# pwrliang/grpc-rdma

Hardware: NVIDIA B200
Metric: streaming_payload_GBps_256conns_4MiB (higher is better)
Workload: dtype u8

## Files before the change

### grpc-rdma_b200/csrc/b200_dev.cuh

```cuda
#pragma once
#include <stdint.h>

#if defined(__CUDACC__)
#define B200_HD __host__ __device__ __forceinline__
#else
#define B200_HD inline
#endif

namespace b200 {

constexpr uint64_t kAlign = 8;
constexpr uint64_t kReserved = 24;
constexpr uint64_t kFooter = ~0ull;
constexpr int kMaxSgeLimit = 32;

B200_HD uint64_t round_up8(uint64_t v) { return (v + 7) & ~7ull; }
B200_HD uint64_t round_down8(uint64_t v) { return v & ~7ull; }
B200_HD uint64_t encoded_size(uint64_t payload) { return 16 + round_up8(payload); }
B200_HD uint64_t calc_writable(uint64_t space) { return space > kReserved ? round_down8(space - kReserved) : 0; }
B200_HD uint64_t free_size(uint64_t cap, uint64_t head, uint64_t tail) {
  return cap - ((tail + cap - head) & (cap - 1));
}
B200_HD uint64_t writable_size(uint64_t cap, uint64_t head, uint64_t tail) {
  uint64_t f = free_size(cap, head, tail);
  return f > kReserved ? f - kReserved : 0;
}

struct PairMirror {
  uint64_t head, moving_head, remain, acc;
  uint64_t remote_tail, credit_head;
  uint64_t readable;
  uint32_t partial_write;
  uint32_t peer_exit;
  uint32_t has_message;
  uint32_t _reserved;
};

struct __align__(128) PairDev {
  uint8_t* ring;
  uint64_t cap;
  uint8_t* peer_ring;
  uint64_t* peer_credit;
  PairMirror* mirror;
  PairMirror* peer_mirror;
  uint32_t status;
  uint32_t max_sge;
  int32_t peer_slot;
  uint32_t wire;
  uint64_t head;
  uint64_t moving_head;
  uint64_t remain;
  uint64_t acc;
  uint64_t remote_tail;
  uint32_t partial_write;
  uint32_t mlock;
  uint64_t credit_head;
  uint32_t credit_exit;
  uint32_t _pad1;
};
static_assert(sizeof(PairDev) == 128, "PairDev is one 128-byte line");

struct SliceDev {
  const uint8_t* ptr;
  uint64_t len;
};

struct SendOpDev {
  int32_t slot;
  uint32_t flags;
  const SliceDev* slices;
  uint64_t nslices;
  uint64_t byte_idx;
  uint64_t nreal;
};

struct RecvOpDev {
  int32_t slot;
  uint32_t flags;
  uint8_t* dst;
  uint64_t cap;
};

struct OpResult {
  uint64_t bytes;
  uint64_t calls;
};

constexpr uint32_t kFlagUntilBlocked = 0x1;
constexpr uint32_t kFlagConcurrent = 0x8;
constexpr uint32_t kEvReadable = 0x1;
constexpr uint32_t kEvWritable = 0x4;

constexpr uint32_t kStConnected = 2;
constexpr uint32_t kStHalfClosed = 3;
constexpr uint32_t kStError = 5;

constexpr uint32_t kSvcSend = 1, kSvcRecv = 2, kSvcStop = 3, kSvcRetire = 4, kSvcNop = 5;
constexpr uint32_t kSvcInline = 5;
constexpr uint32_t kOwnQ = 16;
constexpr uint32_t kOwnBoxes = 8;
constexpr uint32_t kSmallMax = 8192;
constexpr uint32_t kEagerMax = 2048;
constexpr uint32_t kSvcSliceArea = 1024;
struct __align__(128) SvcCmd {
  uint32_t stamp;
  uint32_t op;
  int32_t slot;
  uint32_t flags;
  uint64_t ptr;
  uint64_t n;
  uint64_t byte_idx;
  SliceDev inl[kSvcInline];
  uint32_t nreal;
  uint32_t stamp2;
};
static_assert(sizeof(SvcCmd) == 128, "one command = one 128-byte line");
struct __align__(16) SvcDone {
  uint64_t bytes;
  uint32_t calls;
  uint32_t seq;
};
static_assert(sizeof(SvcDone) == 16, "one answer = one 16-byte store");
struct PairSvc {
  uint64_t delivered;
  uint64_t pushed_at;
};
struct __align__(32) EagerRec {
  uint64_t at;
  uint64_t csum;
  uint32_t size;
  uint32_t magic;
  uint64_t _pad;
};
constexpr uint32_t kEagerMagic = 0xEA6E7001u;
struct __align__(128) BigBox {
  uint32_t state;
  uint32_t kind;
  int32_t slot;
  uint32_t flags;
  uint64_t ptr, n, byte_idx, nreal;
  SliceDev inl[kSvcInline];
  SvcDone* done;
  uint32_t seq;
  uint32_t _pad;
  OpResult res;
};
B200_HD uint64_t eager_mix(uint64_t x) {
  x ^= x >> 32;
  x *= 0xD6E8FEB86659FD93ull;
  x ^= x >> 32;
  return x;
}
B200_HD uint64_t eager_word(uint64_t w, uint32_t j) { return eager_mix(w + (uint64_t)(j + 1) * 0x9E3779B97F4A7C15ull); }

constexpr uint32_t kReadyRing = 4096;
struct ReadyEntry {
  uint32_t stamp;
  uint16_t slot;
  uint16_t events;
};
struct SvcPollState {
  uint32_t hi_slot;
  uint32_t stop;
  uint32_t ready_next;
  uint32_t scans;
};
struct SvcParams {
  PairDev* pairs;
  PairSvc* psvc;
  SvcCmd* cmds;
  SvcDone* done;
  BigBox* boxes;
  EagerRec* erec;
  uint8_t* eslots;
  SvcPollState* ps;
  uint32_t* last_ev;
  ReadyEntry* ready;
  uint32_t* host_scans;
  int nowners, nbig;
};

void launch_send(PairDev* pairs, const SendOpDev* ops, OpResult* results, int nops, void* stream);
void launch_recv(PairDev* pairs, const RecvOpDev* ops, OpResult* results, int nops, void* stream);
void launch_poll_scan(PairDev* pairs, const int32_t* slots, uint32_t* events, uint32_t* ready_count,
                      int32_t* ready_slots, int n, void* stream);

bool launch_service(const SvcParams& sp, void* s_owner, void* s_big, void* s_poll);
int svc_trace_read(unsigned long long* out16);

void launch_probe_copy(uint8_t* dst, const uint8_t* src, uint64_t bytes_per_cta, uint64_t stride, int nctas,
                       int threads, uint32_t mis, uint32_t item_bytes, uint32_t dynamic, void* stream);

}
```

### grpc-rdma_b200/csrc/b200_kernels.cu

```cuda
#include <cuda_runtime.h>
#include <stdint.h>

#include <mutex>

#include "b200_dev.cuh"

#ifndef B200_RECV_PROXY_FENCE
#define B200_RECV_PROXY_FENCE 1
#endif

namespace b200 {


#define VL(x) (*(volatile decltype(x)*)&(x))

__device__ __forceinline__ uint4 ld_stream16(const void* p) {
  uint4 r;
  asm volatile("ld.global.nc.L1::no_allocate.v4.u32 {%0,%1,%2,%3}, [%4];"
               : "=r"(r.x), "=r"(r.y), "=r"(r.z), "=r"(r.w)
               : "l"(p));
  return r;
}
__device__ __forceinline__ uint4 ld_ring16(const void* p) {
  uint4 r;
  asm volatile("ld.global.L1::no_allocate.v4.u32 {%0,%1,%2,%3}, [%4];"
               : "=r"(r.x), "=r"(r.y), "=r"(r.z), "=r"(r.w)
               : "l"(p));
  return r;
}
__device__ __forceinline__ void st_stream16(void* p, uint4 v) {
  asm volatile("st.global.L1::no_allocate.v4.u32 [%0], {%1,%2,%3,%4};" ::"l"(p), "r"(v.x), "r"(v.y), "r"(v.z),
               "r"(v.w)
               : "memory");
}
__device__ __forceinline__ uint64_t ld_acquire_u64(const void* p) {
  uint64_t v;
  asm volatile("ld.acquire.sys.global.u64 %0, [%1];" : "=l"(v) : "l"(p) : "memory");
  return v;
}
__device__ __forceinline__ uint64_t ld_volatile_u64(const void* p) {
  uint64_t v;
  asm volatile("ld.volatile.global.u64 %0, [%1];" : "=l"(v) : "l"(p) : "memory");
  return v;
}

__device__ __forceinline__ uint32_t ld_acquire_u32(const void* p) {
  uint32_t v;
  asm volatile("ld.acquire.sys.global.u32 %0, [%1];" : "=r"(v) : "l"(p) : "memory");
  return v;
}
__device__ __forceinline__ void st_release_v2u64(void* p, uint64_t a, uint64_t b) {
  __threadfence_system();
  asm volatile("st.global.v2.u64 [%0], {%1,%2};" ::"l"(p), "l"(a), "l"(b) : "memory");
}


__device__ __forceinline__ uint32_t smem_u32(const void* p) { return (uint32_t)__cvta_generic_to_shared(p); }
__device__ __forceinline__ void mbar_init(uint64_t* bar, uint32_t count) {
  asm volatile("mbarrier.init.shared::cta.b64 [%0], %1;" ::"r"(smem_u32(bar)), "r"(count) : "memory");
}
__device__ __forceinline__ void mbar_expect_tx(uint64_t* bar, uint32_t bytes) {
  asm volatile("mbarrier.arrive.expect_tx.shared::cta.b64 _, [%0], %1;" ::"r"(smem_u32(bar)), "r"(bytes) : "memory");
}
__device__ __forceinline__ bool mbar_try_wait(uint64_t* bar, uint32_t parity) {
  uint32_t ok;
  asm volatile(
      "{\n\t.reg .pred p;\n\t"
      "mbarrier.try_wait.parity.shared::cta.b64 p, [%1], %2;\n\t"
      "selp.u32 %0, 1, 0, p;\n\t}"
      : "=r"(ok)
      : "r"(smem_u32(bar)), "r"(parity)
      : "memory");
  return ok != 0;
}
__device__ __forceinline__ void bulk_g2s(void* sdst, const void* gsrc, uint32_t bytes, uint64_t* bar) {
  asm volatile("cp.async.bulk.shared::cluster.global.mbarrier::complete_tx::bytes [%0], [%1], %2, [%3];" ::"r"(
                   smem_u32(sdst)),
               "l"(gsrc), "r"(bytes), "r"(smem_u32(bar))
               : "memory");
}
__device__ __forceinline__ void fence_proxy_async_global() { asm volatile("fence.proxy.async.global;" ::: "memory"); }

template <int K>
__device__ __forceinline__ void s2g_vectors(uint4* __restrict__ dv, const uint4* __restrict__ sv, uint32_t nvec,
                                            uint32_t r, uint32_t lane) {
#pragma unroll 4
  for (uint32_t i = lane; i < nvec; i += 32) {
    const uint4 A = sv[i], B = sv[i + 1];
    uint32_t x0, x1, x2, x3, x4;
    if (K == 0) { x0 = A.x; x1 = A.y; x2 = A.z; x3 = A.w; x4 = B.x; }
    else if (K == 1) { x0 = A.y; x1 = A.z; x2 = A.w; x3 = B.x; x4 = B.y; }
    else if (K == 2) { x0 = A.z; x1 = A.w; x2 = B.x; x3 = B.y; x4 = B.z; }
    else { x0 = A.w; x1 = B.x; x2 = B.y; x3 = B.z; x4 = B.w; }
    uint4 o;
    o.x = __funnelshift_r(x0, x1, r);
    o.y = __funnelshift_r(x1, x2, r);
    o.z = __funnelshift_r(x2, x3, r);
    o.w = __funnelshift_r(x3, x4, r);
    st_stream16(dv + i, o);
  }
}

__device__ __forceinline__ void smem_to_global(uint8_t* dst, const uint8_t* sbase, uint32_t soff, uint32_t n,
                                               uint32_t lane) {
  if (n == 0) return;
  uint32_t head = (16 - (uint32_t)(reinterpret_cast<uintptr_t>(dst) & 15)) & 15;
  if (head > n) head = n;
  const uint32_t nvec = (n - head) >> 4;
  const uint32_t tail = n - head - (nvec << 4);
  if (lane < head) dst[lane] = sbase[soff + lane];
  if (lane < tail) dst[head + (nvec << 4) + lane] = sbase[soff + head + (nvec << 4) + lane];
  const uint32_t vs = soff + head, m = vs & 15;
  const uint4* sv = reinterpret_cast<const uint4*>(sbase + (vs - m));
  uint4* dv = reinterpret_cast<uint4*>(dst + head);
  if (m == 0) {
#pragma unroll 4
    for (uint32_t i = lane; i < nvec; i += 32) st_stream16(dv + i, sv[i]);
    return;
  }
  const uint32_t r = (m & 3) * 8;
  switch (m >> 2) {
    case 0: s2g_vectors<0>(dv, sv, nvec, r, lane); break;
    case 1: s2g_vectors<1>(dv, sv, nvec, r, lane); break;
    case 2: s2g_vectors<2>(dv, sv, nvec, r, lane); break;
    default: s2g_vectors<3>(dv, sv, nvec, r, lane); break;
  }
}

__device__ __forceinline__ void coop_zero(uint8_t* p, uint64_t n, uint32_t lane) {
  if (n == 0) return;
  uint64_t head = (16 - (reinterpret_cast<uintptr_t>(p) & 15)) & 15;
  if (head > n) head = n;
  if (lane < head) p[lane] = 0;
  p += head;
  n -= head;
  const uint64_t nvec = n >> 4;
  uint4* d = reinterpret_cast<uint4*>(p);
  const uint4 z = make_uint4(0, 0, 0, 0);
  for (uint64_t i = lane; i < nvec; i += 32) st_stream16(d + i, z);
  const uint64_t done = nvec << 4;
  if (lane < n - done) p[done + lane] = 0;
}

template <bool kSys = true>
__device__ __forceinline__ void rx_probe(const uint8_t* ring, uint64_t cap, uint64_t head, uint64_t remain,
                                         uint32_t& has_msg, uint64_t& readable) {
  if (remain > 0) {
    has_msg = 1;
    readable = remain;
    return;
  }
  uint64_t hdr = kSys ? ld_acquire_u64(ring + head) : ld_volatile_u64(ring + head);
  has_msg = hdr != 0;
  readable = 0;
  if (hdr != 0 && hdr <= cap - kReserved) {
    const uint8_t* fp = ring + ((head + 8 + round_up8(hdr)) & (cap - 1));
    uint64_t foot = kSys ? ld_acquire_u64(fp) : ld_volatile_u64(fp);
    if (foot == kFooter) readable = hdr;
  }
}

__device__ __forceinline__ void publish_mirror_rx(PairMirror* m, const PairDev* P, uint32_t has_msg,
                                                  uint64_t readable) {
  if (m == nullptr) return;
  volatile PairMirror* vm = m;
  vm->head = P->head;
  vm->moving_head = P->moving_head;
  vm->remain = P->remain;
  vm->acc = P->acc;
  vm->readable = readable;
  vm->has_message = has_msg;
}
__device__ __forceinline__ void publish_mirror_tx(PairMirror* m, const PairDev* P) {
  if (m == nullptr) return;
  volatile PairMirror* vm = m;
  vm->remote_tail = P->remote_tail;
  vm->credit_head = *(volatile const uint64_t*)&P->credit_head;
  vm->partial_write = P->partial_write;
  vm->peer_exit = *(volatile const uint32_t*)&P->credit_exit;
}

__device__ __forceinline__ void mirror_lock(PairDev* P, bool on) {
  if (!on) return;
  while (atomicCAS(&P->mlock, 0u, 1u) != 0u) __nanosleep(64);
  __threadfence();
}
__device__ __forceinline__ void mirror_unlock(PairDev* P, bool on) {
  if (!on) return;
  __threadfence_system();
  atomicExch(&P->mlock, 0u);
}


#ifndef B200_MOVERS
#define B200_MOVERS 8
#endif
#ifndef B200_DEPTH
#define B200_DEPTH 3
#endif
#ifndef B200_CHUNK
#define B200_CHUNK 4096
#endif
constexpr int kMovers = B200_MOVERS;
constexpr int kThreads = 32 * (1 + kMovers);
constexpr int kDepth = B200_DEPTH;
constexpr uint32_t kChunk = B200_CHUNK;
constexpr uint32_t kStageBytes = kChunk + 32;
constexpr uint32_t kStageTotal = kMovers * kDepth * kStageBytes;
constexpr uint32_t kQI = 128;

struct WorkItem {
  uint64_t a;
  uint64_t b;
  uint64_t c;
  uint32_t n;
  uint32_t ready;
};

struct PipeCtl {
  uint32_t next;
  uint32_t total_items;
  uint32_t seg_done;
  uint32_t op_done;
};

__device__ __forceinline__ uint32_t ld_shared_volatile(const uint32_t* p) { return *(const volatile uint32_t*)p; }

__device__ __forceinline__ void publish_item(WorkItem* q, uint32_t id, uint64_t a, uint64_t b, uint64_t c,
                                             uint32_t n) {
  WorkItem* slot = &q[id % kQI];
  while (ld_shared_volatile(&slot->ready) != 0) __nanosleep(20);
  slot->a = a;
  slot->b = b;
  slot->c = c;
  slot->n = n;
  __threadfence_block();
  *(volatile uint32_t*)&slot->ready = id + 1;
}

__device__ __forceinline__ void movers_init(uint64_t* bars, uint32_t tid) {
  if (tid < kMovers * kDepth) mbar_init(&bars[tid], 1);
  asm volatile("fence.mbarrier_init.release.cluster;" ::: "memory");
  asm volatile("fence.proxy.async.shared::cta;" ::: "memory");
}

template <class Move>
__device__ __forceinline__ void mover_run(const Move& mv, WorkItem* q, PipeCtl* ctl, uint8_t* stages, uint64_t* bars,
                                          uint32_t& phase_bits, uint32_t lane) {
  static_assert(kQI <= 256 && kDepth <= 8, "slot_of packs one byte per stage");
  uint32_t head = 0, tail = 0, ticket = 0;
  uint64_t slot_of = 0;
  bool drained = false;
  if (lane == 0) ticket = atomicAdd(&ctl->next, 1u);
  while (true) {
    while (!drained && tail - head < (uint32_t)kDepth) {
      uint32_t st = 0;
      if (lane == 0) {
        const uint32_t si = ticket % kQI;
        WorkItem* slot = &q[si];
        if (ld_shared_volatile(&slot->ready) == ticket + 1) {
          st = 1;
        } else if (ld_shared_volatile(&ctl->seg_done) && ticket >= ld_shared_volatile(&ctl->total_items)) {
          st = ld_shared_volatile(&slot->ready) == ticket + 1 ? 1 : 2;
        }
        if (st == 1) {
          __threadfence_block();
          const uint32_t s = tail % kDepth;
          mv.issue(slot->a, slot->n, stages + s * kStageBytes, &bars[s]);
          st |= si << 8;
          ticket = atomicAdd(&ctl->next, 1u);
        }
      }
      st = __shfl_sync(0xffffffffu, st, 0);
      if ((st & 3) == 1) {
        const uint32_t sh = 8 * (tail % kDepth);
        slot_of = (slot_of & ~(0xffull << sh)) | ((uint64_t)(st >> 8) << sh);
        tail++;
      } else {
        drained = (st & 3) == 2;
        break;
      }
    }
    __syncwarp();
    if (head == tail) {
      if (drained) break;
      __nanosleep(32);
      continue;
    }
    const uint32_t s = head % kDepth;
    const uint32_t par = (phase_bits >> s) & 1u;
    while (!mbar_try_wait(&bars[s], par)) {
    }
    phase_bits ^= 1u << s;
    WorkItem* w = &q[(uint32_t)(slot_of >> (8 * s)) & 0xffu];
    const uint64_t ia = w->a, ib = w->b, ic = w->c;
    const uint32_t in = w->n;
    mv.process(ia, ib, ic, in, stages + s * kStageBytes, lane);
    __syncwarp();
    if (lane == 0) *(volatile uint32_t*)&w->ready = 0;
    head++;
  }
}


constexpr uint32_t kTiny = 32;
constexpr uint32_t kFootCap = 1024;

struct SendPlanState {
  uint64_t rt, cap, staging, total_left, written_total, ncalls, cur, bidx, last_rh;
  uint32_t partial, max_sge;
};

struct SendCallScratch {
  const uint8_t* src[kMaxSgeLimit];
  uint64_t len[kMaxSgeLimit];
  uint64_t off[kMaxSgeLimit];
  uint32_t first_item[kMaxSgeLimit + 1];
};

__device__ __noinline__ void send_produce_segment(const SendOpDev& op, const PairDev* P, uint8_t* ring,
                                                  SendPlanState& S, SendCallScratch& CS, WorkItem* q, PipeCtl* ctl,
                                                  uint32_t* foot8, uint32_t* nfoot_out, uint32_t lane) {
  const uint64_t cap = S.cap, mask = cap - 1;
  uint32_t base_item = 0, nfoot = 0;
  bool op_done = false;
  while (nfoot + kMaxSgeLimit <= kFootCap) {
    const uint64_t rt = S.rt;
    const uint64_t rh = ld_volatile_u64(&P->credit_head);
    if (rh != S.last_rh) {
      if (P->wire != 0) __threadfence_system();
      else __threadfence();
      S.last_rh = rh;
    }
    const uint64_t cur = S.cur, bidx = S.bidx;
    const uint64_t idx = cur + lane;
    const bool valid = lane < S.max_sge && idx < op.nreal;
    const uint8_t* ptr = nullptr;
    uint64_t len = 0;
    if (valid) {
      SliceDev sl = op.slices[idx];
      const uint64_t skip = lane == 0 ? bidx : 0;
      ptr = sl.ptr + skip;
      len = sl.len - skip;
    }
    const uint64_t e = valid ? encoded_size(len) : 0;
    uint64_t incl = e;
    for (int o = 1; o < 32; o <<= 1) {
      uint64_t t = __shfl_up_sync(0xffffffffu, incl, o);
      if (lane >= (uint32_t)o) incl += t;
    }
    const uint64_t a = incl - e;
    const uint64_t fr = free_size(cap, rh, rt);
    const uint64_t lim = S.staging < fr ? S.staging : fr;
    const uint64_t room = calc_writable(lim > a ? lim - a : 0);
    const bool fits = valid && len != 0 && len <= room;
    const unsigned bad = __ballot_sync(0xffffffffu, !fits);
    const int first_bad = __ffs(bad) - 1;
    const int nfull = first_bad < 0 ? 32 : first_bad;
    uint64_t p = 0;
    if ((int)lane < nfull) p = len;
    else if ((int)lane == nfull && valid && len != 0) p = room;
    const unsigned fmask = __ballot_sync(0xffffffffu, p != 0);
    const uint32_t nframes = __popc(fmask);
    uint64_t wsum = p, esum = p ? encoded_size(p) : 0;
    const bool tiny = p != 0 && p <= kTiny;
    const uint32_t items = (p && !tiny) ? (uint32_t)((p + kChunk - 1) / kChunk) : 0;
    uint32_t items_incl = items;
    for (int o = 1; o < 32; o <<= 1) {
      uint32_t t = __shfl_up_sync(0xffffffffu, items_incl, o);
      if (lane >= (uint32_t)o) items_incl += t;
    }
    for (int o = 16; o > 0; o >>= 1) {
      wsum += __shfl_xor_sync(0xffffffffu, wsum, o);
      esum += __shfl_xor_sync(0xffffffffu, esum, o);
    }
    const uint32_t nitems = __shfl_sync(0xffffffffu, items_incl, 31);
    const uint64_t cut_p = __shfl_sync(0xffffffffu, p, nfull < 32 ? nfull : 0);
    const uint64_t foff = (rt + a) & mask;
    CS.first_item[lane] = items_incl - items;
    if (p) {
      CS.src[lane] = ptr;
      CS.len[lane] = p;
      CS.off[lane] = foff;
      foot8[nfoot + lane] = (uint32_t)(((foff + 8 + round_up8(p)) & mask) >> 3);
    }
    if (tiny) {
      uint64_t w[kTiny / 8];
#pragma unroll
      for (int k = 0; k < (int)(kTiny / 8); k++) w[k] = 0;
#pragma unroll
      for (int i = 0; i < (int)kTiny; i++)
        if ((uint64_t)i < p) w[i >> 3] |= (uint64_t)__ldg(ptr + i) << (8 * (i & 7));
      *reinterpret_cast<uint64_t*>(ring + foff) = p;
#pragma unroll
      for (int k = 0; k < (int)(kTiny / 8); k++)
        if ((uint64_t)(8 * k) < p) *reinterpret_cast<uint64_t*>(ring + ((foff + 8 + 8 * k) & mask)) = w[k];
    }
    if (lane == 0) {
      CS.first_item[32] = nitems;
      S.rt = (rt + esum) & mask;
      S.partial = wsum < S.total_left;
      S.total_left -= wsum;
      S.written_total += wsum;
      if (wsum) S.ncalls++;
      uint64_t nb = 0;
      if (nfull < 32 && nframes > (uint32_t)nfull) nb = (nfull == 0 ? bidx : 0) + cut_p;
      else if (nfull == 0) nb = bidx;
      S.cur = cur + nfull;
      S.bidx = nb;
    }
    __syncwarp();
    nfoot += nframes;
    const unsigned big = __ballot_sync(0xffffffffu, items > 8);
    if (!big && nitems <= kQI) {
      const uint32_t first = items_incl - items;
      for (uint32_t t = 0; t < items; t++) {
        const uint64_t c0 = (uint64_t)t * kChunk;
        uint64_t n = p - c0;
        if (n > kChunk) n = kChunk;
        publish_item(q, base_item + first + t, reinterpret_cast<uint64_t>(ptr + c0), (foff + 8 + c0) & mask,
                     c0 == 0 ? p : 0, (uint32_t)n);
      }
    } else
    for (uint32_t it = lane; it < nitems; it += 32) {
      uint32_t f = 0;
      while (f + 1 < nframes && CS.first_item[f + 1] <= it) f++;
      const uint64_t c0 = (uint64_t)(it - CS.first_item[f]) * kChunk;
      const uint64_t flen = CS.len[f];
      uint64_t n = flen - c0;
      if (n > kChunk) n = kChunk;
      publish_item(q, base_item + it, reinterpret_cast<uint64_t>(CS.src[f] + c0), (CS.off[f] + 8 + c0) & mask,
                   c0 == 0 ? flen : 0, (uint32_t)n);
    }
    __syncwarp();
    base_item += nitems;
    const bool last = (wsum == 0) || !(op.flags & kFlagUntilBlocked) || S.total_left == 0;
    if (last) {
      op_done = true;
      break;
    }
  }
  if (lane == 0) {
    *nfoot_out = nfoot;
    ctl->total_items = base_item;
    ctl->op_done = op_done ? 1u : 0u;
    __threadfence_block();
    *(volatile uint32_t*)&ctl->seg_done = 1;
  }
  __syncwarp();
}

struct SendMove {
  uint8_t* ring;
  uint64_t cap, mask;
  __device__ __forceinline__ void issue(uint64_t a, uint32_t n, uint8_t* stage, uint64_t* bar) const {
    const uint32_t pre = (uint32_t)(a & 15);
    const uint32_t len = (pre + n + 15u) & ~15u;
    mbar_expect_tx(bar, len);
    bulk_g2s(stage, reinterpret_cast<const void*>(a - pre), len, bar);
  }
  __device__ __forceinline__ void process(uint64_t a, uint64_t b, uint64_t c, uint32_t n, const uint8_t* stage,
                                          uint32_t lane) const {
    const uint32_t pre = (uint32_t)(a & 15);
    if (c != 0 && lane == 0) *reinterpret_cast<uint64_t*>(ring + ((b + cap - 8) & mask)) = c;
    uint64_t seg1 = cap - b;
    if (seg1 > n) seg1 = n;
    smem_to_global(ring + b, stage, pre, (uint32_t)seg1, lane);
    if (n > seg1) smem_to_global(ring, stage, pre + (uint32_t)seg1, n - (uint32_t)seg1, lane);
  }
};

struct PipeSmem {
  WorkItem q[kQI];
  PipeCtl ctl;
  uint64_t bars[kMovers * kDepth];
};

__device__ __forceinline__ void send_body(PairDev* __restrict__ pairs, const SendOpDev& op, OpResult* result,
                                          PipeSmem& pipe, uint8_t* stage_mem, uint32_t& phase_bits) {
  WorkItem* q = pipe.q;
  PipeCtl& ctl = pipe.ctl;
  uint64_t* bars = pipe.bars;
  __shared__ SendPlanState PS;
  __shared__ SendCallScratch CS;
  __shared__ uint32_t foot8[kFootCap];
  __shared__ uint32_t s_nfoot;
  __shared__ unsigned long long s_total;
  __shared__ uint32_t s_status;
  PairDev* P = &pairs[op.slot];
  const uint32_t tid = threadIdx.x, lane = tid & 31, warp = tid >> 5;

  if (tid < kQI) q[tid].ready = 0;
  if (tid == 0) {
    s_total = 0;
    s_status = *(volatile uint32_t*)&P->status;
    PS.rt = *(volatile uint64_t*)&P->remote_tail;
    PS.cap = *(volatile uint64_t*)&P->cap;
    PS.staging = PS.cap / 2;
    PS.max_sge = *(volatile uint32_t*)&P->max_sge;
    PS.cur = 0;
    PS.bidx = op.byte_idx;
    PS.written_total = 0;
    PS.ncalls = 0;
    PS.partial = *(volatile uint32_t*)&P->partial_write;
    PS.last_rh = ~0ull;
  }
  __syncthreads();
  {
    unsigned long long part = 0;
    for (uint64_t i = tid; i < op.nslices; i += kThreads) part += op.slices[i].len;
    for (int o = 16; o > 0; o >>= 1) part += __shfl_down_sync(0xffffffffu, part, o);
    if (lane == 0 && part) atomicAdd(&s_total, part);
  }
  __syncthreads();
  if (s_status != kStConnected) {
    if (tid == 0) {
      result->bytes = 0;
      result->calls = 0;
    }
    return;
  }
  if (tid == 0) PS.total_left = s_total - op.byte_idx;
  const uint64_t cap = VL(P->cap), mask = cap - 1;
  uint8_t* ring = VL(P->peer_ring);
  const bool sys_scope = VL(P->wire) != 0;

  while (true) {
    if (tid == 0) {
      ctl.next = 0;
      ctl.total_items = 0;
      ctl.seg_done = 0;
      ctl.op_done = 0;
      s_nfoot = 0;
    }
    __syncthreads();
    if (warp == 0) {
      send_produce_segment(op, P, ring, PS, CS, q, &ctl, foot8, &s_nfoot, lane);
    } else {
      const SendMove mv{ring, cap, mask};
      mover_run(mv, q, &ctl, stage_mem + (warp - 1) * (kDepth * kStageBytes), &bars[(warp - 1) * kDepth], phase_bits, lane);
    }
    if (sys_scope) __threadfence_system();
    else __threadfence();
    __syncthreads();
    const uint32_t nfoot = s_nfoot;
    for (uint32_t i = tid; i < nfoot; i += kThreads)
      *reinterpret_cast<uint64_t*>(ring + ((uint64_t)foot8[i] << 3)) = kFooter;
    const bool done = ctl.op_done != 0;
    __syncthreads();
    if (done) break;
  }
  if (tid == 0) {
    P->remote_tail = PS.rt;
    P->partial_write = PS.partial;
    result->bytes = PS.written_total;
    result->calls = PS.ncalls;
    const bool conc = (op.flags & kFlagConcurrent) != 0;
    mirror_lock(P, conc);
    publish_mirror_tx(VL(P->mirror), P);
    mirror_unlock(P, conc);
    const int peer_slot = VL(P->peer_slot);
    if (peer_slot >= 0 && PS.written_total) {
      PairDev* Q = &pairs[peer_slot];
      PairMirror* qm = VL(Q->mirror);
      if (qm) {
        uint32_t hm;
        uint64_t rd;
        mirror_lock(Q, conc);
        rx_probe<false>(VL(Q->ring), VL(Q->cap), *(volatile uint64_t*)&Q->head, *(volatile uint64_t*)&Q->remain, hm, rd);
        volatile PairMirror* vm = qm;
        vm->has_message = hm;
        vm->readable = rd;
        mirror_unlock(Q, conc);
      }
    }
  }
}

__global__ void __launch_bounds__(kThreads, 2)
k_send(PairDev* __restrict__ pairs, const SendOpDev* __restrict__ ops, OpResult* __restrict__ results) {
  extern __shared__ __align__(128) uint8_t stage_mem[];
  __shared__ PipeSmem pipe;
  movers_init(pipe.bars, threadIdx.x);
  uint32_t phase_bits = 0;
  const SendOpDev op = ops[blockIdx.x];
  send_body(pairs, op, &results[blockIdx.x], pipe, stage_mem, phase_bits);
}


struct ScoutState {
  uint64_t head, mh, remain, acc, cap_left, delivered, ncalls;
  uint64_t credit_val;
  uint32_t credit_flag;
};

__device__ __noinline__ void recv_produce_segment(const RecvOpDev& op, const uint8_t* ring, uint64_t cap,
                                                  ScoutState& SS, WorkItem* q, PipeCtl* ctl, uint32_t lane) {
  const uint64_t mask = cap - 1;
  uint64_t head = SS.head, mh = SS.mh, remain = SS.remain, acc = SS.acc, cap_left = SS.cap_left;
  uint64_t delivered = SS.delivered, ncalls = SS.ncalls;
  uint64_t win = 0, win_base = 0;
  bool win_valid = false;
  uint32_t base_item = 0, credit = 0, last = 0;
  uint64_t credit_val = 0;
  uint64_t last_reload = 0;
  bool have_last = false;
  auto peek = [&](uint64_t off) -> uint64_t {
    uint64_t d = (off - win_base) & mask;
    if (!win_valid || d >= 256) {
      if (have_last) {
        const uint64_t stride = (off - last_reload) & mask;
        if (stride >= 256) {
          const uint64_t pf = (off + (uint64_t)((lane & 15) + 1) * stride + (lane >> 4) * 128) & mask;
          asm volatile("prefetch.global.L2 [%0];" ::"l"(ring + pf));
        }
      }
      last_reload = off;
      have_last = true;
      win_base = off;
      win = ld_volatile_u64(ring + ((off + 8ull * lane) & mask));
      win_valid = true;
      d = 0;
    }
    return __shfl_sync(0xffffffffu, win, (int)(d >> 3));
  };
  const bool one_call = !(op.flags & kFlagUntilBlocked);
  uint32_t pstate = 0;
  uint64_t pe1 = 0, pe2 = 0;
  while (true) {
    uint64_t my_r = 0, my_head = 0;
    bool my_open = false;
    uint32_t cnt = 0;
    bool stopped = false, predicted = false;
    uint64_t h = head;
    if (remain > 0) {
      if (lane == 0) my_r = remain;
      cnt = 1;
    }
    if (!one_call && pstate == 1) {
      predicted = true;
      const uint32_t c0 = cnt;
      const uint32_t j = lane - c0;
      const uint64_t pred_e = (j & 1) ? pe1 : pe2;
      const uint64_t rel = (uint64_t)(j >> 1) * (pe1 + pe2) + ((j & 1) ? pe2 : 0);
      const bool mine = lane >= c0 && rel + pred_e <= cap;
      const uint64_t off = (h + rel) & mask;
      uint64_t hdr = 0;
      if (mine) hdr = ld_volatile_u64(ring + off);
      const uint64_t e = 16 + round_up8(hdr);
      const bool valid = mine && hdr != 0 && hdr <= cap - kReserved && rel + e <= cap;
      const unsigned mism = __ballot_sync(0xffffffffu, lane >= c0 && !(valid && e == pred_e));
      const uint32_t k = mism ? (uint32_t)__ffs(mism) - 1 : 32u;
      uint64_t foot = 0;
      if (valid && lane <= k) foot = ld_volatile_u64(ring + ((off + 8 + round_up8(hdr)) & mask));
      const bool complete = valid && lane <= k && foot == kFooter;
      const unsigned inc = __ballot_sync(0xffffffffu, lane >= c0 && !complete);
      const uint32_t stop_lane = inc ? (uint32_t)__ffs(inc) - 1 : 32u;
      if (lane >= c0 && lane < stop_lane) {
        my_r = hdr;
        my_head = off;
        my_open = true;
      }
      stopped = stop_lane < 32 && stop_lane <= k && ((__ballot_sync(0xffffffffu, mine) >> stop_lane) & 1u);
      cnt = stop_lane;
      if (cnt > c0) {
        const uint64_t off_l = __shfl_sync(0xffffffffu, off, cnt - 1);
        const uint64_t e_l = __shfl_sync(0xffffffffu, e, cnt - 1);
        h = (off_l + e_l) & mask;
      }
      if (!stopped && cnt - c0 < 4) pstate = 2;
    } else {
      const uint32_t want = one_call ? 1u : (pstate == 0 ? cnt + 2u : 32u);
      while (cnt < want) {
        const uint64_t hdr = peek(h);
        if (hdr == 0 || hdr > cap - kReserved) { stopped = true; break; }
        const uint64_t foot = peek((h + 8 + round_up8(hdr)) & mask);
        if (foot != kFooter) { stopped = true; break; }
        if (lane == cnt) {
          my_r = hdr;
          my_head = h;
          my_open = true;
        }
        h = (h + 16 + round_up8(hdr)) & mask;
        cnt++;
      }
    }
    const bool valid = lane < cnt;
    uint64_t r_incl = valid ? my_r : 0;
    for (int o = 1; o < 32; o <<= 1) {
      uint64_t t = __shfl_up_sync(0xffffffffu, r_incl, o);
      if (lane >= (uint32_t)o) r_incl += t;
    }
    const uint64_t r_excl = r_incl - (valid ? my_r : 0);
    const uint64_t room = cap_left > r_excl ? cap_left - r_excl : 0;
    const uint64_t n = valid ? (my_r < room ? my_r : room) : 0;
    const bool full = valid && n == my_r && n != 0;
    const unsigned notfull = __ballot_sync(0xffffffffu, !full);
    const int first_nf = __ffs(notfull) - 1;
    uint32_t nproc = first_nf < 0 ? 32u : (uint32_t)first_nf;
    {
      const uint64_t n_at = __shfl_sync(0xffffffffu, n, nproc < 32 ? nproc : 0);
      if (nproc < 32 && n_at != 0) nproc++;
    }
    const uint64_t src = my_open ? (my_head + 8) & mask : mh;
    const uint64_t end = (src + n) & mask;
    uint32_t ztail = 0;
    uint64_t mh_after = end;
    if (n == my_r) {
      const uint64_t up = round_up8(end);
      ztail = (uint32_t)(up - end) + 8;
      mh_after = ((up & mask) + 8) & mask;
    }
    const uint32_t zhead = my_open ? 8u : 0u;
    const bool proc = lane < nproc;
    uint64_t a_incl = proc ? (uint64_t)zhead + n + ztail : 0;
    for (int o = 1; o < 32; o <<= 1) {
      uint64_t t = __shfl_up_sync(0xffffffffu, a_incl, o);
      if (lane >= (uint32_t)o) a_incl += t;
    }
    const unsigned cross = __ballot_sync(0xffffffffu, proc && acc + a_incl >= cap / 2);
    if (cross) {
      const uint32_t ci = (uint32_t)__ffs(cross) - 1;
      nproc = ci + 1;
      credit = 1;
      credit_val = __shfl_sync(0xffffffffu, mh_after, ci);
    }
    if (nproc == 0) {
      last = 1;
      break;
    }
    const bool proc2 = lane < nproc;
    const bool tiny = proc2 && my_open && n == my_r && n <= kTiny;
    if (tiny) {
      uint64_t w[kTiny / 8];
#pragma unroll
      for (int k = 0; k < (int)(kTiny / 8); k++)
        w[k] = (uint64_t)(8 * k) < n ? ld_volatile_u64(ring + ((my_head + 8 + 8 * k) & mask)) : 0;
      uint8_t* d = op.dst + delivered + r_excl;
#pragma unroll
      for (int i = 0; i < (int)kTiny; i++)
        if ((uint64_t)i < n) d[i] = (uint8_t)(w[i >> 3] >> (8 * (i & 7)));
      uint8_t* wr = const_cast<uint8_t*>(ring);
      const uint32_t nw = (uint32_t)(round_up8(n) >> 3) + 2;
      for (uint32_t k = 0; k < nw; k++) *reinterpret_cast<uint64_t*>(wr + ((my_head + 8 * k) & mask)) = 0;
    }
    const uint32_t items = (proc2 && !tiny) ? (uint32_t)((n + kChunk - 1) / kChunk) : 0;
    uint32_t items_incl = items;
    for (int o = 1; o < 32; o <<= 1) {
      uint32_t t = __shfl_up_sync(0xffffffffu, items_incl, o);
      if (lane >= (uint32_t)o) items_incl += t;
    }
    const uint32_t nitems = __shfl_sync(0xffffffffu, items_incl, 31);
    const uint32_t my_first = items_incl - items;
    for (uint32_t it0 = 0; it0 < nitems; it0 += 32) {
      const uint32_t it = it0 + lane;
      uint32_t f = 0;
      for (uint32_t g = 0; g < nproc; g++) {
        const uint32_t fg = __shfl_sync(0xffffffffu, my_first, g);
        const uint32_t ig = __shfl_sync(0xffffffffu, items, g);
        if (ig && fg <= it) f = g;
      }
      const uint64_t f_src = __shfl_sync(0xffffffffu, src, f);
      const uint64_t f_n = __shfl_sync(0xffffffffu, n, f);
      const uint64_t f_dst = delivered + __shfl_sync(0xffffffffu, r_excl, f);
      const uint32_t f_first = __shfl_sync(0xffffffffu, my_first, f);
      const uint32_t f_zh = __shfl_sync(0xffffffffu, zhead, f);
      const uint32_t f_zt = __shfl_sync(0xffffffffu, ztail, f);
      if (it < nitems) {
        const uint64_t c0 = (uint64_t)(it - f_first) * kChunk;
        uint64_t m = f_n - c0;
        const bool tail_item = m <= kChunk;
        if (m > kChunk) m = kChunk;
        const uint64_t z = (c0 == 0 ? f_zh : 0u) | ((uint64_t)(tail_item ? f_zt : 0u) << 16);
        publish_item(q, base_item + it, (f_src + c0) & mask, f_dst + c0, z, (uint32_t)m);
      }
    }
    __syncwarp();
    base_item += nitems;
    const uint32_t L = nproc - 1;
    const bool open_L = __shfl_sync(0xffffffffu, (int)my_open, L) != 0;
    const uint64_t head_L = __shfl_sync(0xffffffffu, my_head, L);
    const uint64_t r_L = __shfl_sync(0xffffffffu, my_r, L);
    const uint64_t n_L = __shfl_sync(0xffffffffu, n, L);
    const uint64_t moved = __shfl_sync(0xffffffffu, r_excl, L) + n_L;
    if (open_L) head = (head_L + 16 + round_up8(r_L)) & mask;
    mh = __shfl_sync(0xffffffffu, mh_after, L);
    remain = r_L - n_L;
    acc = credit ? 0 : acc + __shfl_sync(0xffffffffu, a_incl, L);
    delivered += moved;
    cap_left -= moved;
    ncalls += nproc;
    if (one_call || cap_left == 0 || (stopped && nproc == cnt)) last = 1;
    if (last || credit) break;
    {
      const bool two = L >= 1 && __shfl_sync(0xffffffffu, (int)my_open, L - (L >= 1 ? 1 : 0)) != 0 && open_L && remain == 0;
      if (two) {
        const uint64_t ra = r_L, rb = __shfl_sync(0xffffffffu, my_r, L - 1);
        const uint64_t na = 16 + round_up8(ra), nb = 16 + round_up8(rb);
        bool ok = true;
        if (pstate == 2 && !predicted) {
          ok = false;
          if (L >= 3) {
            const uint64_t rc = __shfl_sync(0xffffffffu, my_r, L - 2), rd = __shfl_sync(0xffffffffu, my_r, L - 3);
            const bool oc = __shfl_sync(0xffffffffu, (int)my_open, L - 3) != 0;
            ok = oc && round_up8(rc) == round_up8(ra) && round_up8(rd) == round_up8(rb);
          }
        }
        pe1 = na;
        pe2 = nb;
        if (pstate == 0 || (pstate == 2 && !predicted && ok)) pstate = 1;
      } else if (pstate == 1) {
        pstate = 0;
      }
    }
  }
  if (lane == 0) {
    SS.head = head;
    SS.mh = mh;
    SS.remain = remain;
    SS.acc = acc;
    SS.cap_left = cap_left;
    SS.delivered = delivered;
    SS.ncalls = ncalls;
    SS.credit_flag = credit;
    SS.credit_val = credit_val;
    ctl->total_items = base_item;
    ctl->op_done = last;
    __threadfence_block();
    *(volatile uint32_t*)&ctl->seg_done = 1;
  }
  __syncwarp();
}

struct RecvMove {
  uint8_t* ring;
  uint8_t* dst;
  uint64_t cap, mask;
  __device__ __forceinline__ void issue(uint64_t a, uint32_t n, uint8_t* stage, uint64_t* bar) const {
    const uint32_t pre = (uint32_t)(a & 15);
    const uint64_t start = a - pre;
#if B200_RECV_PROXY_FENCE
    fence_proxy_async_global();
#endif
    if (a + n <= cap) {
      const uint32_t len = (pre + n + 15u) & ~15u;
      mbar_expect_tx(bar, len);
      bulk_g2s(stage, ring + start, len, bar);
    } else {
      const uint32_t len1 = (uint32_t)(cap - start);
      const uint32_t n2 = n - (uint32_t)(cap - a);
      const uint32_t len2 = (n2 + 15u) & ~15u;
      mbar_expect_tx(bar, len1 + len2);
      bulk_g2s(stage, ring + start, len1, bar);
      bulk_g2s(stage + len1, ring, len2, bar);
    }
  }
  __device__ __forceinline__ void process(uint64_t a, uint64_t b, uint64_t c, uint32_t n, const uint8_t* stage,
                                          uint32_t lane) const {
    const uint32_t zhead = (uint32_t)(c & 0xffff), ztail = (uint32_t)(c >> 16);
    const uint64_t zs = (a + cap - zhead) & mask;
    const uint64_t zl = (uint64_t)zhead + n + ztail;
    uint64_t z1 = cap - zs;
    if (z1 > zl) z1 = zl;
    coop_zero(ring + zs, z1, lane);
    if (zl > z1) coop_zero(ring, zl - z1, lane);
    smem_to_global(dst + b, stage, (uint32_t)(a & 15), n, lane);
  }
};

__device__ __forceinline__ void recv_body(PairDev* __restrict__ pairs, const RecvOpDev& op, OpResult* result,
                                          PipeSmem& pipe, uint8_t* stage_mem, uint32_t& phase_bits) {
  WorkItem* q = pipe.q;
  PipeCtl& ctl = pipe.ctl;
  uint64_t* bars = pipe.bars;
  __shared__ ScoutState SS;
  __shared__ uint32_t s_status;
  PairDev* P = &pairs[op.slot];
  const uint32_t tid = threadIdx.x, lane = tid & 31, warp = tid >> 5;

  if (tid < kQI) q[tid].ready = 0;
  if (tid == 0) {
    s_status = *(volatile uint32_t*)&P->status;
    SS.head = *(volatile uint64_t*)&P->head;
    SS.mh = *(volatile uint64_t*)&P->moving_head;
    SS.remain = *(volatile uint64_t*)&P->remain;
    SS.acc = *(volatile uint64_t*)&P->acc;
    SS.cap_left = op.cap;
    SS.delivered = 0;
    SS.ncalls = 0;
    SS.credit_flag = 0;
  }
  __syncthreads();
  if (s_status != kStConnected) {
    if (tid == 0) {
      result->bytes = 0;
      result->calls = 0;
    }
    return;
  }
  uint8_t* ring = VL(P->ring);
  const uint64_t cap = VL(P->cap), mask = cap - 1;

  while (true) {
    if (tid == 0) {
      ctl.next = 0;
      ctl.total_items = 0;
      ctl.seg_done = 0;
      ctl.op_done = 0;
    }
    __syncthreads();
    if (warp == 0) {
      recv_produce_segment(op, ring, cap, SS, q, &ctl, lane);
    } else {
      const RecvMove mv{ring, op.dst, cap, mask};
      mover_run(mv, q, &ctl, stage_mem + (warp - 1) * (kDepth * kStageBytes), &bars[(warp - 1) * kDepth], phase_bits, lane);
    }
    const bool credit = ld_shared_volatile(&SS.credit_flag) != 0;
    if (credit) __threadfence_system();
    __syncthreads();
    const bool done = ctl.op_done != 0;
    if (tid == 0 && credit) {
      const int peer_slot = VL(P->peer_slot);
      const bool conc = (op.flags & kFlagConcurrent) != 0 && peer_slot >= 0;
      PairDev* Q = conc ? &pairs[peer_slot] : nullptr;
      if (conc) mirror_lock(Q, true);
      st_release_v2u64(VL(P->peer_credit), SS.credit_val, 0);
      PairMirror* pm = VL(P->peer_mirror);
      if (pm) ((volatile PairMirror*)pm)->credit_head = SS.credit_val;
      if (conc) mirror_unlock(Q, true);
      SS.credit_flag = 0;
    }
    __syncthreads();
    if (done) break;
  }
  if (tid == 0) {
    P->head = SS.head;
    P->moving_head = SS.mh;
    P->remain = SS.remain;
    P->acc = SS.acc;
    result->bytes = SS.delivered;
    result->calls = SS.ncalls;
    uint32_t hm;
    uint64_t rd;
    const bool conc = (op.flags & kFlagConcurrent) != 0;
    mirror_lock(P, conc);
    rx_probe<false>(ring, cap, SS.head, SS.remain, hm, rd);
    publish_mirror_rx(VL(P->mirror), P, hm, rd);
    mirror_unlock(P, conc);
  }
}

__global__ void __launch_bounds__(kThreads, 2)
k_recv(PairDev* __restrict__ pairs, const RecvOpDev* __restrict__ ops, OpResult* __restrict__ results) {
  extern __shared__ __align__(128) uint8_t stage_mem[];
  __shared__ PipeSmem pipe;
  movers_init(pipe.bars, threadIdx.x);
  uint32_t phase_bits = 0;
  const RecvOpDev op = ops[blockIdx.x];
  recv_body(pairs, op, &results[blockIdx.x], pipe, stage_mem, phase_bits);
}


__global__ void __launch_bounds__(128)
k_poll_scan(PairDev* __restrict__ pairs, const int32_t* __restrict__ slots, uint32_t* __restrict__ events,
            uint32_t* __restrict__ ready_count, int32_t* __restrict__ ready_slots, int n) {
  const int i = blockIdx.x * blockDim.x + threadIdx.x;
  const uint32_t lane = threadIdx.x & 31;
  uint32_t ev = 0;
  int32_t slot = -1;
  if (i < n) {
    slot = slots[i];
    PairDev* P = &pairs[slot];
    const uint32_t st = *(volatile uint32_t*)&P->status;
    if (st == kStConnected) {
      const uint32_t exit_flag = ld_acquire_u32(&P->credit_exit);
      uint32_t hm;
      uint64_t rd;
      rx_probe(P->ring, P->cap, *(volatile uint64_t*)&P->head, *(volatile uint64_t*)&P->remain, hm, rd);
      const uint32_t pw = *(volatile uint32_t*)&P->partial_write;
      if (exit_flag == 1) {
        ev = kEvReadable;
      } else {
        if (hm) ev |= kEvReadable;
        if (pw) ev |= kEvWritable;
      }
      if (P->peer_slot < 0) {
        publish_mirror_rx(P->mirror, P, hm, rd);
        publish_mirror_tx(P->mirror, P);
      }
    } else if (st == kStError || st == kStHalfClosed) {
      ev = kEvReadable;
    }
    events[i] = ev;
  }
  const unsigned m = __ballot_sync(0xffffffffu, ev != 0);
  if (m) {
    uint32_t base = 0;
    if (lane == (uint32_t)(__ffs(m) - 1)) base = atomicAdd(ready_count, __popc(m));
    base = __shfl_sync(0xffffffffu, base, __ffs(m) - 1);
    if (ev) ready_slots[base + __popc(m & ((1u << lane) - 1))] = slot;
  }
}


__device__ __forceinline__ uint64_t ld_sys_u64(const void* p) {
  uint64_t v;
  asm volatile("ld.relaxed.sys.global.u64 %0, [%1];" : "=l"(v) : "l"(p) : "memory");
  return v;
}
__device__ __forceinline__ uint4 ld_sys_v4(const void* p) {
  uint4 r;
  asm volatile("ld.relaxed.sys.global.v4.u32 {%0,%1,%2,%3}, [%4];"
               : "=r"(r.x), "=r"(r.y), "=r"(r.z), "=r"(r.w)
               : "l"(p)
               : "memory");
  return r;
}
__device__ __forceinline__ void st_sys_v4(void* p, uint4 v) {
  asm volatile("st.relaxed.sys.global.v4.u32 [%0], {%1,%2,%3,%4};" ::"l"(p), "r"(v.x), "r"(v.y), "r"(v.z), "r"(v.w)
               : "memory");
}
__device__ __forceinline__ void st_sys_u64(void* p, uint64_t v) {
  asm volatile("st.relaxed.sys.global.u64 [%0], %1;" ::"l"(p), "l"(v) : "memory");
}
__device__ __forceinline__ uint8_t ld_volatile_u8(const void* p) { return *(const volatile uint8_t*)p; }

#ifdef B200_SVC_TRACE
__device__ unsigned long long g_svc_trace[16];
__device__ __forceinline__ unsigned long long gtime() {
  unsigned long long t;
  asm volatile("mov.u64 %0, %%globaltimer;" : "=l"(t));
  return t;
}
#define TRACE_MARK(i, t0) do { if (lane == 0) atomicAdd(&g_svc_trace[i], gtime() - (t0)); } while (0)
#else
#define TRACE_MARK(i, t0) do { } while (0)
#endif


constexpr int kCopyBatch = 8;

__device__ __forceinline__ uint64_t warp_copy_to_ring(uint8_t* ring, uint64_t mask, uint64_t off, const uint8_t* src,
                                                      uint32_t n, uint8_t* eslot, uint32_t lane) {
  const uintptr_t s = reinterpret_cast<uintptr_t>(src);
  const uint32_t sb = (uint32_t)(s & 7), sh = sb * 8;
  const uint64_t* s0 = reinterpret_cast<const uint64_t*>(s & ~(uintptr_t)7);
  const uint32_t words = (n + 7) >> 3;
  uint64_t cs = 0;
  for (uint32_t base = 0; base < words; base += 32 * kCopyBatch) {
    uint64_t lo[kCopyBatch], hi[kCopyBatch];
#pragma unroll
    for (int k = 0; k < kCopyBatch; k++) {
      const uint32_t j = base + 32 * k + lane;
      lo[k] = j < words ? ld_sys_u64(s0 + j) : 0;
    }
    if (sh) {
#pragma unroll
      for (int k = 0; k < kCopyBatch; k++) {
        const uint32_t j = base + 32 * k + lane;
        const uint32_t lastb = (8 * j + 8 < n ? 8 * j + 8 : n) - 1;
        hi[k] = (j < words && (sb + lastb) / 8 > j) ? ld_sys_u64(s0 + j + 1) : 0;
      }
    }
#pragma unroll
    for (int k = 0; k < kCopyBatch; k++) {
      const uint32_t j = base + 32 * k + lane;
      if (j < words) {
        uint64_t w = sh ? (lo[k] >> sh) | (hi[k] << (64 - sh)) : lo[k];
        const uint32_t rem = n - 8 * j;
        if (rem < 8) w &= (1ull << (8 * rem)) - 1;
        *reinterpret_cast<uint64_t*>(ring + ((off + 8ull * j) & mask)) = w;
        if (eslot) {
          st_sys_u64(eslot + 8ull * j, w);
          cs ^= eager_word(w, j);
        }
      }
    }
  }
  return cs;
}

__device__ __forceinline__ void warp_copy_from_ring(uint8_t* dst, const uint8_t* ring, uint64_t mask, uint64_t off,
                                                    uint32_t n, uint32_t lane) {
  const uintptr_t d = reinterpret_cast<uintptr_t>(dst);
  uint32_t head = (uint32_t)((8 - (d & 7)) & 7);
  if (head > n) head = n;
  if (lane < head) dst[lane] = ld_volatile_u8(ring + ((off + lane) & mask));
  const uint32_t nwords = (n - head) >> 3;
  const uint64_t o = off + head;
  const uint32_t sh = (uint32_t)(o & 7) * 8;
  const uint64_t o0 = o & ~7ull;
  for (uint32_t base = 0; base < nwords; base += 32 * kCopyBatch) {
    uint64_t lo[kCopyBatch], hi[kCopyBatch];
#pragma unroll
    for (int k = 0; k < kCopyBatch; k++) {
      const uint32_t j = base + 32 * k + lane;
      lo[k] = j < nwords ? ld_volatile_u64(ring + ((o0 + 8ull * j) & mask)) : 0;
    }
    if (sh) {
#pragma unroll
      for (int k = 0; k < kCopyBatch; k++) {
        const uint32_t j = base + 32 * k + lane;
        hi[k] = j < nwords ? ld_volatile_u64(ring + ((o0 + 8ull * j + 8) & mask)) : 0;
      }
    }
#pragma unroll
    for (int k = 0; k < kCopyBatch; k++) {
      const uint32_t j = base + 32 * k + lane;
      if (j < nwords) *reinterpret_cast<uint64_t*>(dst + head + 8ull * j) = sh ? (lo[k] >> sh) | (hi[k] << (64 - sh)) : lo[k];
    }
  }
  const uint32_t tail = n - head - 8 * nwords;
  if (lane < tail) dst[head + 8 * nwords + lane] = ld_volatile_u8(ring + ((o + 8ull * nwords + lane) & mask));
}

__device__ __forceinline__ void warp_zero_ring(uint8_t* ring, uint64_t mask, uint64_t zs, uint64_t zl, uint32_t lane) {
  uint64_t head = (8 - (zs & 7)) & 7;
  if (head > zl) head = zl;
  if (lane < head) ring[(zs + lane) & mask] = 0;
  const uint64_t nwords = (zl - head) >> 3;
  const uint64_t o = zs + head;
  for (uint64_t k = lane; k < nwords; k += 32) *reinterpret_cast<uint64_t*>(ring + ((o + 8 * k) & mask)) = 0;
  const uint64_t tail = zl - head - 8 * nwords;
  if (lane < tail) ring[(o + 8 * nwords + lane) & mask] = 0;
}

constexpr int kConnCache = 8;
struct ConnEntry {
  PairDev line[2];
  PairSvc svc[2];
  int32_t slot[2];
};
struct ConnView {
  PairDev* P;
  PairDev* Q;
  PairSvc* SP;
  PairSvc* SQ;
};

__device__ __forceinline__ ConnView conn_get(ConnEntry* cc, uint32_t& cc_next, const SvcParams& sp, int pslot,
                                             int peer_hint, uint32_t lane) {
  int hit = -1, side = 0;
  {
    bool mine = false;
    int myside = 0;
    if (lane < kConnCache) {
      if (cc[lane].slot[0] == pslot) mine = true, myside = 0;
      else if (cc[lane].slot[1] == pslot) mine = true, myside = 1;
    }
    const unsigned m = __ballot_sync(0xffffffffu, mine);
    if (m) {
      hit = __ffs(m) - 1;
      side = __shfl_sync(0xffffffffu, myside, hit);
    }
  }
  if (hit < 0) {
    hit = (int)(cc_next % kConnCache);
    cc_next++;
    side = 0;
    ConnEntry& e = cc[hit];
    uint4 v = make_uint4(0, 0, 0, 0);
    if (lane < 8) v = ld_sys_v4(reinterpret_cast<const uint4*>(&sp.pairs[pslot]) + lane);
    else if (lane < 16 && peer_hint >= 0) v = ld_sys_v4(reinterpret_cast<const uint4*>(&sp.pairs[peer_hint]) + (lane - 8));
    else if (lane == 16) v = ld_sys_v4(reinterpret_cast<const uint4*>(&sp.psvc[pslot]));
    else if (lane == 17 && peer_hint >= 0) v = ld_sys_v4(reinterpret_cast<const uint4*>(&sp.psvc[peer_hint]));
    if (lane < 8) reinterpret_cast<uint4*>(&e.line[0])[lane] = v;
    else if (lane < 16) reinterpret_cast<uint4*>(&e.line[1])[lane - 8] = v;
    else if (lane == 16) *reinterpret_cast<uint4*>(&e.svc[0]) = v;
    else if (lane == 17) *reinterpret_cast<uint4*>(&e.svc[1]) = v;
    __syncwarp();
    int peer = e.line[0].peer_slot;
    if (peer != peer_hint) {
      if (lane < 8 && peer >= 0) reinterpret_cast<uint4*>(&e.line[1])[lane] = ld_sys_v4(reinterpret_cast<const uint4*>(&sp.pairs[peer]) + lane);
      if (lane == 8 && peer >= 0) *reinterpret_cast<uint4*>(&e.svc[1]) = ld_sys_v4(reinterpret_cast<const uint4*>(&sp.psvc[peer]));
      __syncwarp();
    }
    if (lane == 0) {
      e.slot[0] = pslot;
      e.slot[1] = peer;
    }
    __syncwarp();
  }
  ConnEntry& e = cc[hit];
  ConnView v;
  v.P = &e.line[side];
  v.SP = &e.svc[side];
  const bool has_q = e.slot[side ^ 1] >= 0 && e.slot[side ^ 1] == e.line[side].peer_slot;
  v.Q = has_q ? &e.line[side ^ 1] : nullptr;
  v.SQ = has_q ? &e.svc[side ^ 1] : nullptr;
  return v;
}

__device__ __forceinline__ void conn_drop(ConnEntry* cc, int pslot, uint32_t lane) {
  if (lane < kConnCache && (cc[lane].slot[0] == pslot || cc[lane].slot[1] == pslot)) cc[lane].slot[0] = cc[lane].slot[1] = -1;
  __syncwarp();
}
__device__ __forceinline__ void conn_drop_all(ConnEntry* cc, uint32_t lane) {
  if (lane < kConnCache) cc[lane].slot[0] = cc[lane].slot[1] = -1;
  __syncwarp();
}

__device__ __forceinline__ void eager_publish(const SvcParams& sp, int qslot, PairSvc* SQ, uint64_t at, uint64_t size,
                                              uint64_t cs, uint32_t lane) {
  for (int o = 16; o > 0; o >>= 1) cs ^= __shfl_xor_sync(0xffffffffu, cs, o);
  cs ^= eager_mix(at * 31 + size);
  if (lane == 0) {
    EagerRec* r = &sp.erec[qslot];
    uint4 a, b;
    a.x = (uint32_t)at; a.y = (uint32_t)(at >> 32); a.z = (uint32_t)cs; a.w = (uint32_t)(cs >> 32);
    b.x = (uint32_t)size; b.y = kEagerMagic; b.z = 0; b.w = 0;
    st_sys_v4(r, a);
    st_sys_v4(reinterpret_cast<uint8_t*>(r) + 16, b);
    SQ->pushed_at = at;
    VL(sp.psvc[qslot].pushed_at) = at;
  }
}

__device__ __forceinline__ void svc_rx_refresh(const SvcParams& sp, const PairDev& Q, int qslot, PairSvc* SQ,
                                               uint64_t head, uint64_t mh, uint64_t remain, uint64_t acc,
                                               bool known_empty, uint32_t lane) {
  const uint64_t cap = Q.cap, mask = cap - 1;
  const uint8_t* ring = Q.ring;
  const uint64_t delivered = SQ->delivered, pushed_at = SQ->pushed_at;
  uint32_t hm = 0;
  uint64_t rd = 0;
  if (remain > 0) {
    hm = 1;
    rd = remain;
  } else if (!known_empty) {
    const uint64_t hdr = ld_volatile_u64(ring + head);
    hm = hdr != 0;
    if (hdr != 0 && hdr <= cap - kReserved) {
      const bool small = hdr <= kEagerMax && sp.erec != nullptr && pushed_at != delivered;
      const uint32_t words = small ? (uint32_t)((hdr + 7) >> 3) : 0;
      uint64_t w[kEagerMax / 8 / 32];
#pragma unroll
      for (int k = 0; k < (int)(kEagerMax / 8 / 32); k++) {
        const uint32_t j = k * 32 + lane;
        w[k] = j < words ? ld_volatile_u64(ring + ((head + 8 + 8ull * j) & mask)) : 0;
      }
      const uint64_t foot = ld_volatile_u64(ring + ((head + 8 + round_up8(hdr)) & mask));
      if (foot == kFooter) {
        rd = hdr;
        if (small) {
          uint8_t* slot = sp.eslots + (size_t)qslot * kEagerMax;
          uint64_t cs = 0;
#pragma unroll
          for (int k = 0; k < (int)(kEagerMax / 8 / 32); k++) {
            const uint32_t j = k * 32 + lane;
            if (j < words) {
              uint64_t x = w[k];
              const uint32_t rem = (uint32_t)hdr - 8 * j;
              if (rem < 8) x &= (1ull << (8 * rem)) - 1;
              st_sys_u64(slot + 8ull * j, x);
              cs ^= eager_word(x, j);
            }
          }
          eager_publish(sp, qslot, SQ, delivered, hdr, cs, lane);
        }
      }
    }
  }
// ... 342 lines not shown
          bx->nreal = c.nreal;
          bx->done = &qdone[(expect - 1) % kOwnQ];
          bx->seq = expect;
          os.box_a[bi] = pslot;
          os.box_b[bi] = peer;
          os.box_kind[bi] = opc == kSvcSend ? kSvcSend : kSvcRecv;
        }
        if (lane < kSvcInline) bx->inl[lane] = c.inl[lane];
        __threadfence();
        __syncwarp();
        if (lane == 0) *(volatile uint32_t*)&bx->state = 1;
        answer = false;
      }
    }
    if (answer) {
      if (opc == kSvcRecv && res.bytes) __threadfence_system();
      __syncwarp();
      if (lane == 0) {
        uint4 d;
        d.x = (uint32_t)res.bytes;
        d.y = (uint32_t)(res.bytes >> 32);
        d.z = (uint32_t)res.calls;
        d.w = expect;
        st_sys_v4(&qdone[(expect - 1) % kOwnQ], d);
      }
      TRACE_MARK(3, tr0);
#ifdef B200_SVC_TRACE
      if (lane == 0) atomicAdd(&g_svc_trace[4], 1ull);
#endif
    }
    expect++;
    cur++;
    avail--;
    __syncwarp();
  }
  for (int i = 0; i < (int)kOwnBoxes; i++) {
    if (lane == 0 && os.box_a[i] >= 0)
      while (*(volatile uint32_t*)&boxes[i].state != 3) __nanosleep(200);
  }
  __syncwarp();
  if (lane == 0) {
    __threadfence_system();
    uint4 d = make_uint4(0, 0, 0, expect);
    st_sys_v4(&qdone[(expect - 1) % kOwnQ], d);
  }
}

__global__ void __launch_bounds__(kThreads, 2) k_svc_big(SvcParams sp) {
  extern __shared__ __align__(128) uint8_t stage_mem[];
  __shared__ PipeSmem pipe;
  __shared__ OpResult s_res;
  __shared__ int s_pick;
  __shared__ uint32_t s_stop;
  __shared__ __align__(16) BigBox s_box;
  const uint32_t tid = threadIdx.x;
  movers_init(pipe.bars, tid);
  uint32_t phase_bits = 0;
  const int nboxes = sp.nowners * (int)kOwnBoxes;
  uint32_t idle = 0;
  while (true) {
    if (tid == 0) {
      s_pick = 0x7fffffff;
      s_stop = *(volatile uint32_t*)&sp.ps->stop;
    }
    __syncthreads();
    if (s_stop) break;
    for (int i = tid; i < nboxes; i += kThreads) {
      const int b = (i + blockIdx.x * 37) % nboxes;
      if (*(volatile uint32_t*)&sp.boxes[b].state == 1) atomicMin(&s_pick, i);
    }
    __syncthreads();
    int pick = s_pick;
    __syncthreads();
    if (pick != 0x7fffffff) {
      const int b = (pick + blockIdx.x * 37) % nboxes;
      if (tid == 0) s_pick = atomicCAS(&sp.boxes[b].state, 1u, 2u) == 1u ? b : -1;
      __syncthreads();
      pick = s_pick;
      __syncthreads();
    } else {
      pick = -1;
    }
    if (pick < 0) {
      if (++idle > 16) __nanosleep(idle > 4096 ? 2000 : 300);
      continue;
    }
    idle = 0;
    BigBox* bx = &sp.boxes[pick];
    __threadfence();
    if (tid < sizeof(BigBox) / 16) reinterpret_cast<uint4*>(&s_box)[tid] = ld_sys_v4(reinterpret_cast<const uint4*>(bx) + tid);
    if (tid == 0) {
      s_res.bytes = 0;
      s_res.calls = 0;
    }
    __syncthreads();
    const uint32_t kind = s_box.kind;
    if (kind == kSvcSend) {
      SendOpDev op;
      op.slot = s_box.slot;
      op.flags = s_box.flags;
      op.nslices = s_box.n;
      op.slices = op.nslices <= kSvcInline ? s_box.inl : reinterpret_cast<const SliceDev*>(s_box.ptr);
      op.byte_idx = s_box.byte_idx;
      op.nreal = s_box.nreal;
      send_body(sp.pairs, op, &s_res, pipe, stage_mem, phase_bits);
    } else {
      RecvOpDev op;
      op.slot = s_box.slot;
      op.flags = s_box.flags;
      op.dst = reinterpret_cast<uint8_t*>(s_box.ptr);
      op.cap = s_box.n;
      recv_body(sp.pairs, op, &s_res, pipe, stage_mem, phase_bits);
    }
    if (kind == kSvcRecv) __threadfence_system();
    __syncthreads();
    if (tid == 0) {
      bx->res = s_res;
      uint4 d;
      d.x = (uint32_t)s_res.bytes;
      d.y = (uint32_t)(s_res.bytes >> 32);
      d.z = (uint32_t)s_res.calls;
      d.w = s_box.seq;
      st_sys_v4(s_box.done, d);
      __threadfence();
      *(volatile uint32_t*)&bx->state = 3;
    }
    __syncthreads();
  }
}

__device__ __forceinline__ void service_poll_loop(PairDev* pairs, SvcPollState* ps, uint32_t* last_ev,
                                                  ReadyEntry* ready, uint32_t* host_scans) {
  const uint32_t tid = threadIdx.x, lane = tid & 31;
  __shared__ uint32_t s_hi, s_stop;
  while (true) {
    if (tid == 0) {
      s_hi = *(volatile uint32_t*)&ps->hi_slot;
      s_stop = *(volatile uint32_t*)&ps->stop;
    }
    __syncthreads();
    const uint32_t hi = s_hi;
    if (s_stop) break;
    for (uint32_t base = 0; base < hi; base += kThreads) {
      const uint32_t slot = base + tid;
      uint32_t ev = 0, changed = 0;
      if (slot < hi) {
        PairDev* P = &pairs[slot];
        const uint32_t st = *(volatile uint32_t*)&P->status;
        uint32_t hm = 0;
        uint64_t rd = 0;
        if (st == kStConnected) {
          const uint32_t exit_flag = ld_acquire_u32(&P->credit_exit);
          rx_probe(P->ring, P->cap, *(volatile uint64_t*)&P->head, *(volatile uint64_t*)&P->remain, hm, rd);
          const uint32_t pw = *(volatile uint32_t*)&P->partial_write;
          if (exit_flag == 1) {
            ev = kEvReadable;
          } else {
            if (hm) ev |= kEvReadable;
            if (pw) ev |= kEvWritable;
          }
          ev |= (uint32_t)(rd != 0) << 8;
        } else if (st == kStError || st == kStHalfClosed) {
          ev = kEvReadable;
        }
        changed = ev != last_ev[slot];
        if (changed) {
          last_ev[slot] = ev;
          if (st == kStConnected && P->peer_slot < 0) {
            publish_mirror_rx(P->mirror, P, hm, rd);
            publish_mirror_tx(P->mirror, P);
          }
        }
      }
      const unsigned m = __ballot_sync(0xffffffffu, changed != 0);
      if (m) {
        const int leader = __ffs(m) - 1;
        uint32_t idx = 0;
        if ((int)lane == leader) idx = atomicAdd(&ps->ready_next, (uint32_t)__popc(m));
        idx = __shfl_sync(0xffffffffu, idx, leader) + __popc(m & ((1u << lane) - 1));
        if (changed) {
          __threadfence_system();
          ReadyEntry e;
          e.stamp = idx + 1;
          e.slot = (uint16_t)slot;
          e.events = (uint16_t)(ev & 0xff);
          *reinterpret_cast<volatile uint64_t*>(&ready[idx % kReadyRing]) = *reinterpret_cast<uint64_t*>(&e);
        }
      }
    }
    __syncthreads();
    if (tid == 0) {
      const uint32_t n = ++ps->scans;
      if ((n & 1023u) == 0) *(volatile uint32_t*)host_scans = n;
    }
    __nanosleep(200);
  }
}

__global__ void __launch_bounds__(kThreads) k_svc_poll(SvcParams sp) {
  service_poll_loop(sp.pairs, sp.ps, sp.last_ev, sp.ready, sp.host_scans);
}

__global__ void __launch_bounds__(kThreads, 2)
k_probe_copy(uint8_t* __restrict__ dst, uint8_t* __restrict__ src, uint64_t bytes_per_cta, uint64_t stride,
             uint32_t mis, uint32_t item_bytes, uint32_t mode) {
  extern __shared__ __align__(128) uint8_t stage_mem[];
  __shared__ PipeSmem pipe;
  WorkItem* q = pipe.q;
  PipeCtl& ctl = pipe.ctl;
  uint64_t* bars = pipe.bars;
  const uint32_t tid = threadIdx.x, lane = tid & 31, warp = tid >> 5;
  uint8_t* d = dst + (uint64_t)blockIdx.x * stride;
  uint8_t* sbase = src + (uint64_t)blockIdx.x * stride;
  uint8_t* sp = sbase + mis;
  if (item_bytes > kChunk) item_bytes = kChunk;
  const uint32_t nitems = (uint32_t)(bytes_per_cta / item_bytes);
  if (tid < kQI) q[tid].ready = 0;
  movers_init(bars, tid);
  uint32_t phase_bits = 0;
  if (tid == 0) {
    ctl.next = 0;
    ctl.total_items = 0;
    ctl.seg_done = 0;
    ctl.op_done = 0;
  }
  __syncthreads();
  const bool zero_after = (mode & 2) != 0;
  constexpr uint64_t kBig = 1ull << 62;
  if (warp == 0) {
    for (uint32_t it = lane; it < nitems; it += 32) {
      const uint64_t off = (uint64_t)it * item_bytes;
      publish_item(q, it, zero_after ? off + mis : reinterpret_cast<uint64_t>(sp + off), off, 0, item_bytes);
    }
    __syncwarp();
    if (lane == 0) {
      ctl.total_items = nitems;
      __threadfence_block();
      *(volatile uint32_t*)&ctl.seg_done = 1;
    }
  } else if (zero_after) {
    const RecvMove mv{sbase, d, kBig, kBig - 1};
    mover_run(mv, q, &ctl, stage_mem + (warp - 1) * (kDepth * kStageBytes), &bars[(warp - 1) * kDepth], phase_bits, lane);
  } else {
    const SendMove mv{d, kBig, kBig - 1};
    mover_run(mv, q, &ctl, stage_mem + (warp - 1) * (kDepth * kStageBytes), &bars[(warp - 1) * kDepth], phase_bits, lane);
  }
}

static void ensure_kernel_attrs() {
  static std::once_flag once;
  std::call_once(once, [] {
  cudaFuncSetAttribute(k_send, cudaFuncAttributeMaxDynamicSharedMemorySize, (int)kStageTotal);
  cudaFuncSetAttribute(k_recv, cudaFuncAttributeMaxDynamicSharedMemorySize, (int)kStageTotal);
  cudaFuncSetAttribute(k_probe_copy, cudaFuncAttributeMaxDynamicSharedMemorySize, (int)kStageTotal);
  cudaFuncSetAttribute(k_send, cudaFuncAttributePreferredSharedMemoryCarveout, 100);
  cudaFuncSetAttribute(k_recv, cudaFuncAttributePreferredSharedMemoryCarveout, 100);
  cudaFuncSetAttribute(k_probe_copy, cudaFuncAttributePreferredSharedMemoryCarveout, 100);
  cudaFuncSetAttribute(k_svc_big, cudaFuncAttributeMaxDynamicSharedMemorySize, (int)kStageTotal);
  cudaFuncSetAttribute(k_svc_big, cudaFuncAttributePreferredSharedMemoryCarveout, 100);
  cudaFuncAttributes fa;
  cudaFuncGetAttributes(&fa, k_send);
  cudaFuncGetAttributes(&fa, k_recv);
  cudaFuncGetAttributes(&fa, k_poll_scan);
  cudaFuncGetAttributes(&fa, k_probe_copy);
  cudaFuncGetAttributes(&fa, k_svc_owner);
  cudaFuncGetAttributes(&fa, k_svc_big);
  cudaFuncGetAttributes(&fa, k_svc_poll);
  });
}

int svc_trace_read(unsigned long long* out16) {
#ifdef B200_SVC_TRACE
  return cudaMemcpyFromSymbol(out16, g_svc_trace, sizeof(unsigned long long) * 16) == cudaSuccess ? 0 : -1;
#else
  (void)out16;
  return -1;
#endif
}

bool launch_service(const SvcParams& sp, void* s_owner, void* s_big, void* s_poll) {
  ensure_kernel_attrs();
  int dev = 0, sms = 0, per_sm = 0;
  cudaGetDevice(&dev);
  cudaDeviceGetAttribute(&sms, cudaDevAttrMultiProcessorCount, dev);
  if (cudaOccupancyMaxActiveBlocksPerMultiprocessor(&per_sm, k_svc_big, kThreads, kStageTotal) != cudaSuccess ||
      sp.nbig + 2 > per_sm * sms)
    return false;
  const int octas = (sp.nowners + 3) / 4;
  k_svc_owner<<<octas, 128, 0, static_cast<cudaStream_t>(s_owner)>>>(sp);
  k_svc_big<<<sp.nbig, kThreads, kStageTotal, static_cast<cudaStream_t>(s_big)>>>(sp);
  k_svc_poll<<<1, kThreads, 0, static_cast<cudaStream_t>(s_poll)>>>(sp);
  return cudaGetLastError() == cudaSuccess;
}

void launch_probe_copy(uint8_t* dst, const uint8_t* src, uint64_t bytes_per_cta, uint64_t stride, int nctas,
                       int threads, uint32_t mis, uint32_t item_bytes, uint32_t dynamic, void* stream) {
  (void)threads;
  ensure_kernel_attrs();
  k_probe_copy<<<nctas, kThreads, kStageTotal, static_cast<cudaStream_t>(stream)>>>(
      dst, const_cast<uint8_t*>(src), bytes_per_cta, stride, mis, item_bytes, dynamic);
}


void launch_send(PairDev* pairs, const SendOpDev* ops, OpResult* results, int nops, void* stream) {
  if (nops <= 0) return;
  ensure_kernel_attrs();
  k_send<<<nops, kThreads, kStageTotal, static_cast<cudaStream_t>(stream)>>>(pairs, ops, results);
}
void launch_recv(PairDev* pairs, const RecvOpDev* ops, OpResult* results, int nops, void* stream) {
  if (nops <= 0) return;
  ensure_kernel_attrs();
  k_recv<<<nops, kThreads, kStageTotal, static_cast<cudaStream_t>(stream)>>>(pairs, ops, results);
}
void launch_poll_scan(PairDev* pairs, const int32_t* slots, uint32_t* events, uint32_t* ready_count,
                      int32_t* ready_slots, int n, void* stream) {
  if (n <= 0) return;
  ensure_kernel_attrs();
  k_poll_scan<<<(n + 127) / 128, 128, 0, static_cast<cudaStream_t>(stream)>>>(pairs, slots, events, ready_count,
                                                                               ready_slots, n);
}

}
```

### grpc-rdma_b200/csrc/b200_runtime.cu

```cuda
#include <cuda_runtime.h>
#include <errno.h>
#include <poll.h>
#include <stdio.h>
#include <stdlib.h>
#include <string.h>
#include <fcntl.h>
#include <signal.h>
#include <sys/eventfd.h>
#include <sys/stat.h>
#include <unistd.h>

#include <atomic>
#include <chrono>
#include <condition_variable>
#include <map>
#include <mutex>
#include <queue>
#include <string>
#include <thread>
#include <unordered_map>
#include <vector>

#include "../../include/b200_pair.h"
#include "b200_dev.cuh"

using namespace b200;


static thread_local std::string t_err;
static void set_err(const std::string& s) { t_err = s; }
#define CU_OK(call)                                                                      \
  ([&]() -> bool {                                                                       \
    cudaError_t e__ = (call);                                                            \
    if (e__ != cudaSuccess) {                                                            \
      set_err(std::string(#call) + ": " + cudaGetErrorString(e__));                      \
      return false;                                                                      \
    }                                                                                    \
    return true;                                                                         \
  }())


struct Config {
  uint64_t ring_bytes = 4096ull * 1024;
  int poller_threads = 1;
  int busy_poll_us = 500;
  int poller_sleep_ms = 1000;
  int max_sge = 30;
};

struct AddrBlob {
  uint32_t lid;
  uint32_t qpn;
  uint32_t psn;
  uint32_t _pad0;
  uint8_t gid[16];
  uint32_t tag;
  uint32_t _pad1;
  uint64_t ring_buffer_size;
};
static_assert(sizeof(AddrBlob) == B200_ADDRESS_BYTES, "address blob must stay 48 bytes");

struct b200_pair {
  int slot = -1;
  int status = B200_UNINITIALIZED;
  std::string id, error;
  uint8_t* ring = nullptr;
  uint64_t cap = 0;
  int wakeup_fd = -1;
  PairMirror* mirror = nullptr;
  AddrBlob self{};
  AddrBlob peer{};
  b200_pair* peer_local = nullptr;
  bool remote = false;
  uint8_t* remote_ring = nullptr;
  uint64_t* remote_credit = nullptr;
  std::string wire_file;
  bool in_poller = false;
  int peer_pid = 0;
  std::atomic<bool> peer_dead{false};
  std::chrono::steady_clock::time_point last_probe{};
  int max_sge = 30;
  uint64_t svc_delivered = 0;
  std::atomic<bool> retire_pending{false};
  int retire_q = 0;
  uint64_t retire_ticket = 0;
  std::atomic<uint32_t> retire_owed{0};
};

constexpr int kLanes = 16;

struct CopyRun {
  void* dst;
  const void* src;
  size_t bytes;
};

struct LanePlan {
  int first_op = 0, nops = 0;
  std::vector<CopyRun> copies;
};

struct b200_batch {
  int kind = 0;
  int nops = 0;
  int flags = 0;
  void* d_ops = nullptr;
  SliceDev* d_slices = nullptr;
  OpResult* d_results = nullptr;
  OpResult* h_results = nullptr;
  bool staged = false;
  uint8_t* d_stage = nullptr;
  std::vector<int> perm;
  std::vector<b200_pair*> pairs;
  LanePlan lanes[kLanes];
};

static void drain_retire(b200_pair* p);

namespace {

constexpr int kMaxPairs = 8192;

struct Runtime {
  std::mutex mu;
  bool inited = false;
  int dev = -1;
  Config cfg;
  cudaStream_t stream = nullptr;
  cudaStream_t poll_stream = nullptr;
  cudaStream_t lane_up[kLanes] = {}, lane_down[kLanes] = {};
  cudaEvent_t send_done[kLanes] = {}, recv_done[kLanes] = {};
  cudaEvent_t join_up[kLanes] = {}, join_down[kLanes] = {};
  cudaEvent_t fork_event = nullptr;
  PairDev* d_pairs = nullptr;
  PairMirror* h_mirrors = nullptr;
  std::vector<b200_pair*> all_pairs;
  std::queue<b200_pair*> pool;
  std::vector<int> free_slots;
  std::unordered_map<std::string, b200_pair*> id_pair;
  std::map<uint32_t, b200_pair*> by_qpn;
  uint32_t next_qpn = 0x200;
  uint32_t cookie = 0;
  bool ipc_wire = false;
  cudaIpcMemHandle_t pairs_handle{};
  std::map<uint32_t, PairDev*> peer_tables;
  SendOpDev* h_sop = nullptr;
  RecvOpDev* h_rop = nullptr;
  SliceDev* h_slices = nullptr;
  OpResult* h_res = nullptr;
  uint8_t* bounce_tx = nullptr;
  uint8_t* bounce_rx = nullptr;
  uint64_t bounce_tx_cap = 0, bounce_rx_cap = 0;
  std::atomic<uint64_t> launches{0};
  std::mutex pmu;
  std::condition_variable pcv;
  std::vector<b200_pair*> pollables;
  std::vector<std::thread> poll_threads;
  std::atomic<bool> poll_running{false};
  int32_t* h_scan_slots = nullptr;
  uint32_t* h_scan_events = nullptr;
  uint32_t* h_scan_count = nullptr;
  int32_t* h_scan_ready = nullptr;
  std::mutex scan_mu;
  struct OwnerQ {
    std::mutex mu;
    uint64_t next = 0;
  };
  std::atomic<bool> svc_running{false};
  int svc_workers = 0;
  int svc_nowners = 0;
  cudaStream_t svc_stream = nullptr, svc_stream_big = nullptr, svc_stream_poll = nullptr;
  OwnerQ* svc_q = nullptr;
  SvcCmd* svc_cmds = nullptr;
  SvcDone* svc_done = nullptr;
  std::atomic<uint32_t>* svc_consumed = nullptr;
  SliceDev* svc_slices = nullptr;
  EagerRec* svc_erec = nullptr;
  uint8_t* svc_eslots = nullptr;
  BigBox* d_svc_boxes = nullptr;
  PairSvc* d_svc_psvc = nullptr;
  ReadyEntry* svc_ready = nullptr;
  uint32_t* svc_host_scans = nullptr;
  SvcPollState* d_svc_ps = nullptr;
  uint32_t* d_svc_last_ev = nullptr;
  uint32_t svc_hi_slot = 0;
  std::atomic<uint64_t> svc_ops{0}, svc_ready_seen{0}, svc_ready_overflows{0}, svc_eager_hits{0};
  std::atomic<uint32_t> svc_gen{1};
  uint32_t svc_ready_head = 0;
  std::vector<uint16_t> svc_level;
  std::mutex grave_mu;
  std::vector<std::pair<void*, int>> graveyard;
  std::mutex reg_mu;
  std::map<uintptr_t, std::pair<size_t, int>> reg_ranges;
};

Runtime& R() {
  static Runtime r;
  return r;
}

bool ensure_init() {
  if (R().inited) return true;
  return b200_init(-1) == 0;
}

long env_long(const char* k, long dflt) {
  const char* v = getenv(k);
  return v ? atol(v) : dflt;
}

bool is_pow2(uint64_t v) { return v && (v & (v - 1)) == 0; }

bool write_setup(Runtime& r, b200_pair* p, const PairDev& hd) {
  return CU_OK(cudaMemcpyAsync(&r.d_pairs[p->slot], &hd, 64, cudaMemcpyHostToDevice, r.stream)) &&
         CU_OK(cudaStreamSynchronize(r.stream));
}

int reg_kind(const void* p);
int mem_kind3(const void* p) {
  const int k = reg_kind(p);
  if (k) return k;
  cudaPointerAttributes a;
  if (cudaPointerGetAttributes(&a, p) != cudaSuccess) {
    cudaGetLastError();
    return 0;
  }
  if (a.type == cudaMemoryTypeUnregistered) return 0;
  return a.type == cudaMemoryTypeHost ? 1 : 2;
}
int mem_kind(const void* p) { return mem_kind3(p) != 0; }

void kick(b200_pair* p) {
  if (p->wakeup_fd >= 0) (void)eventfd_write(p->wakeup_fd, 1);
}

void rt_free(void* p, int host) {
  if (!p) return;
  Runtime& r = R();
  if (r.svc_running.load()) {
    std::lock_guard<std::mutex> lk(r.grave_mu);
    r.graveyard.push_back({p, host});
    return;
  }
  if (host) cudaFreeHost(p);
  else cudaFree(p);
}

std::atomic<uint64_t> g_reg_epoch{1};
void reg_add(const void* p, size_t n, int kind) {
  Runtime& r = R();
  std::lock_guard<std::mutex> lk(r.reg_mu);
  r.reg_ranges[(uintptr_t)p] = {n, kind};
  g_reg_epoch++;
}
void reg_del(const void* p) {
  Runtime& r = R();
  std::lock_guard<std::mutex> lk(r.reg_mu);
  r.reg_ranges.erase((uintptr_t)p);
  g_reg_epoch++;
}
struct WireDesc {
  uint32_t magic, psn;
  int32_t dev, slot;
  uint64_t cap;
  cudaIpcMemHandle_t ring, pairs;
  int32_t pid, _pad;
};
constexpr uint32_t kWireMagic = 0xB2001BC0u;
std::string wire_path(uint32_t cookie, uint32_t qpn) {
  char b[96];
  snprintf(b, sizeof b, "/dev/shm/b200wire-%08x-%08x", cookie, qpn);
  return b;
}

int reg_kind(const void* p) {
  static thread_local uintptr_t c_base = 0, c_end = 0;
  static thread_local int c_kind = 0;
  static thread_local uint64_t c_epoch = 0;
  const uint64_t ep = g_reg_epoch.load(std::memory_order_acquire);
  if (c_epoch == ep && (uintptr_t)p >= c_base && (uintptr_t)p < c_end) return c_kind;
  Runtime& r = R();
  std::lock_guard<std::mutex> lk(r.reg_mu);
  auto it = r.reg_ranges.upper_bound((uintptr_t)p);
  if (it == r.reg_ranges.begin()) return 0;
  --it;
  if ((uintptr_t)p >= it->first + it->second.first) return 0;
  c_base = it->first;
  c_end = it->first + it->second.first;
  c_kind = it->second.second;
  c_epoch = ep;
  return c_kind;
}

}

struct TlsBounce {
  uint8_t* tx = nullptr;
  uint8_t* rx = nullptr;
  uint64_t tx_cap = 0, rx_cap = 0;
  uint8_t* dstage = nullptr;
  uint64_t dstage_cap = 0;
  cudaStream_t copy_stream = nullptr;
};
static std::mutex g_tls_mu;
static std::vector<TlsBounce*> g_tls_all;
static TlsBounce& tls_bounce() {
  static thread_local TlsBounce* t = nullptr;
  if (!t) {
    t = new TlsBounce();
    std::lock_guard<std::mutex> lk(g_tls_mu);
    g_tls_all.push_back(t);
  }
  return *t;
}


static int init_locked(int device);
extern "C" int b200_init(int device) {
  const bool was = R().inited;
  const int rc = init_locked(device);
  if (rc == 0 && !was) {
    const long n = env_long("B200_SERVICE_AUTOSTART", 0);
    if (n > 0 && b200_service_start((int)n) != 0) return -1;
  }
  return rc;
}
static int init_locked(int device) {
  Runtime& r = R();
  std::lock_guard<std::mutex> lk(r.mu);
  if (r.inited) return 0;
  int ndev = 0;
  if (cudaGetDeviceCount(&ndev) != cudaSuccess || ndev == 0) {
    cudaGetLastError();
    set_err("b200_init: no CUDA device (this library has no CPU fallback)");
    return -1;
  }
  if (device < 0) {
    const char* e = getenv("B200_DEVICE");
    if (e) device = atoi(e);
    else if (cudaGetDevice(&device) != cudaSuccess) device = 0;
  }
  if (!CU_OK(cudaSetDevice(device))) return -1;
  cudaDeviceProp prop;
  if (!CU_OK(cudaGetDeviceProperties(&prop, device))) return -1;
  if (prop.major < 10) {
    set_err("b200_init: device is sm_" + std::to_string(prop.major) + std::to_string(prop.minor) +
            ", this library is built for sm_100a only");
    return -1;
  }
  r.dev = device;
  r.cfg.ring_bytes = (uint64_t)env_long("GRPC_RDMA_RING_BUFFER_SIZE_KB", 4096) * 1024;
  if (getenv("B200_RING_BUFFER_SIZE_BYTES")) r.cfg.ring_bytes = (uint64_t)env_long("B200_RING_BUFFER_SIZE_BYTES", 0);
  r.cfg.poller_threads = (int)env_long("GRPC_RDMA_POLLER_THREAD_NUM", 1);
  r.cfg.busy_poll_us = (int)env_long("GRPC_RDMA_BUSY_POLLING_TIMEOUT_US", 500);
  r.cfg.poller_sleep_ms = (int)env_long("GRPC_RDMA_POLLER_SLEEP_TIMEOUT_MS", 1000);
  r.cfg.max_sge = (int)env_long("GRPC_RDMA_MAX_SGE", 30);
  if (r.cfg.max_sge < 1 || r.cfg.max_sge > kMaxSgeLimit) r.cfg.max_sge = 30;

  if (!CU_OK(cudaStreamCreateWithFlags(&r.stream, cudaStreamNonBlocking))) return -1;
  if (!CU_OK(cudaStreamCreateWithFlags(&r.poll_stream, cudaStreamNonBlocking))) return -1;
  for (int i = 0; i < kLanes; i++) {
    if (!CU_OK(cudaStreamCreateWithFlags(&r.lane_up[i], cudaStreamNonBlocking))) return -1;
    if (!CU_OK(cudaStreamCreateWithFlags(&r.lane_down[i], cudaStreamNonBlocking))) return -1;
    for (cudaEvent_t* e : {&r.send_done[i], &r.recv_done[i], &r.join_up[i], &r.join_down[i]})
      if (!CU_OK(cudaEventCreateWithFlags(e, cudaEventDisableTiming))) return -1;
  }
  if (!CU_OK(cudaEventCreateWithFlags(&r.fork_event, cudaEventDisableTiming))) return -1;
  if (!CU_OK(cudaMalloc(&r.d_pairs, sizeof(PairDev) * kMaxPairs))) return -1;
  if (!CU_OK(cudaMemset(r.d_pairs, 0, sizeof(PairDev) * kMaxPairs))) return -1;
  if (!CU_OK(cudaHostAlloc(&r.h_mirrors, sizeof(PairMirror) * kMaxPairs, cudaHostAllocMapped | cudaHostAllocPortable)))
    return -1;
  memset(r.h_mirrors, 0, sizeof(PairMirror) * kMaxPairs);
  auto halloc = [&](void** p, size_t n) {
    return CU_OK(cudaHostAlloc(p, n, cudaHostAllocMapped | cudaHostAllocPortable));
  };
  if (!halloc((void**)&r.h_sop, sizeof(SendOpDev)) || !halloc((void**)&r.h_rop, sizeof(RecvOpDev)) ||
      !halloc((void**)&r.h_slices, sizeof(SliceDev) * (kMaxSgeLimit + 1)) ||
      !halloc((void**)&r.h_res, sizeof(OpResult)) ||
      !halloc((void**)&r.h_scan_slots, sizeof(int32_t) * kMaxPairs) ||
      !halloc((void**)&r.h_scan_events, sizeof(uint32_t) * kMaxPairs) ||
      !halloc((void**)&r.h_scan_count, sizeof(uint32_t) * 4) ||
      !halloc((void**)&r.h_scan_ready, sizeof(int32_t) * kMaxPairs))
    return -1;
  r.ipc_wire = getenv("B200_IPC_WIRE") ? env_long("B200_IPC_WIRE", 0) != 0 : env_long("WORLD_SIZE", 1) > 1;
  if (r.ipc_wire && !CU_OK(cudaIpcGetMemHandle(&r.pairs_handle, r.d_pairs))) return -1;
  r.free_slots.clear();
  for (int i = kMaxPairs - 1; i >= 0; i--) r.free_slots.push_back(i);
  r.cookie = (uint32_t)getpid() * 2654435761u ^ (uint32_t)(uintptr_t)&r;
  static bool at_exit_registered = false;
  if (!at_exit_registered) {
    at_exit_registered = true;
    atexit([] {
      b200_poller_shutdown();
      b200_service_stop();
      for (b200_pair* p : R().all_pairs)
        if (!p->wire_file.empty()) unlink(p->wire_file.c_str());
    });
  }
  r.inited = true;
  return 0;
}

extern "C" void b200_shutdown(void) {
  b200_poller_shutdown();
  b200_service_stop();
  Runtime& r = R();
  std::lock_guard<std::mutex> lk(r.mu);
  if (!r.inited) return;
  cudaSetDevice(r.dev);
  cudaDeviceSynchronize();
  for (b200_pair* p : r.all_pairs) {
    if (p->ring) cudaFree(p->ring);
    if (p->wakeup_fd >= 0) close(p->wakeup_fd);
    delete p;
  }
  r.all_pairs.clear();
  while (!r.pool.empty()) r.pool.pop();
  r.id_pair.clear();
  r.by_qpn.clear();
  cudaFree(r.d_pairs);
  cudaFreeHost(r.h_mirrors);
  cudaFreeHost(r.h_sop);
  cudaFreeHost(r.h_rop);
  cudaFreeHost(r.h_slices);
  cudaFreeHost(r.h_res);
  cudaFreeHost(r.h_scan_slots);
  cudaFreeHost(r.h_scan_events);
  cudaFreeHost(r.h_scan_count);
  cudaFreeHost(r.h_scan_ready);
  if (r.bounce_tx) cudaFreeHost(r.bounce_tx);
  if (r.bounce_rx) cudaFreeHost(r.bounce_rx);
  {
    std::lock_guard<std::mutex> tl(g_tls_mu);
    for (TlsBounce* t : g_tls_all) {
      if (t->tx) cudaFreeHost(t->tx);
      if (t->rx) cudaFreeHost(t->rx);
      if (t->dstage) cudaFree(t->dstage);
      if (t->copy_stream) cudaStreamDestroy(t->copy_stream);
      t->tx = t->rx = t->dstage = nullptr;
      t->copy_stream = nullptr;
      t->tx_cap = t->rx_cap = t->dstage_cap = 0;
    }
  }
  r.bounce_tx = r.bounce_rx = nullptr;
  r.bounce_tx_cap = r.bounce_rx_cap = 0;
  cudaStreamDestroy(r.stream);
  cudaStreamDestroy(r.poll_stream);
  for (int i = 0; i < kLanes; i++) {
    cudaStreamDestroy(r.lane_up[i]);
    cudaStreamDestroy(r.lane_down[i]);
    for (cudaEvent_t e : {r.send_done[i], r.recv_done[i], r.join_up[i], r.join_down[i]}) cudaEventDestroy(e);
  }
  cudaEventDestroy(r.fork_event);
  r.inited = false;
}

extern "C" int b200_device(void) { return R().dev; }
extern "C" const char* b200_last_error(void) { return t_err.c_str(); }
extern "C" uint64_t b200_launch_count(void) { return R().launches.load(); }

extern "C" int b200_config_set(const char* key, const char* value) {
  if (!ensure_init()) return -1;
  Runtime& r = R();
  std::lock_guard<std::mutex> lk(r.mu);
  std::string k(key);
  long v = atol(value);
  if (k == "GRPC_RDMA_RING_BUFFER_SIZE_KB") {
    if (v <= 0) return -1;
    r.cfg.ring_bytes = (uint64_t)v * 1024;
  } else if (k == "B200_RING_BUFFER_SIZE_BYTES") {
    if (v <= (long)kReserved) return -1;
    r.cfg.ring_bytes = (uint64_t)v;
  } else if (k == "GRPC_RDMA_POLLER_THREAD_NUM") {
    if (v <= 0) return -1;
    r.cfg.poller_threads = (int)v;
  } else if (k == "GRPC_RDMA_BUSY_POLLING_TIMEOUT_US") {
    if (v < 0) return -1;
    r.cfg.busy_poll_us = (int)v;
  } else if (k == "GRPC_RDMA_POLLER_SLEEP_TIMEOUT_MS") {
    if (v < 0) return -1;
    r.cfg.poller_sleep_ms = (int)v;
  } else if (k == "GRPC_RDMA_MAX_SGE") {
    if (v < 1 || v > kMaxSgeLimit) return -1;
    r.cfg.max_sge = (int)v;
  } else {
    set_err("b200_config_set: unknown key " + k);
    return -1;
  }
  return 0;
}

extern "C" int64_t b200_config_get(const char* key) {
  if (!ensure_init()) return -1;
  Runtime& r = R();
  std::string k(key);
  if (k == "GRPC_RDMA_RING_BUFFER_SIZE_KB") return (int64_t)(r.cfg.ring_bytes / 1024);
  if (k == "B200_RING_BUFFER_SIZE_BYTES") return (int64_t)r.cfg.ring_bytes;
  if (k == "GRPC_RDMA_POLLER_THREAD_NUM") return r.cfg.poller_threads;
  if (k == "GRPC_RDMA_BUSY_POLLING_TIMEOUT_US") return r.cfg.busy_poll_us;
  if (k == "GRPC_RDMA_POLLER_SLEEP_TIMEOUT_MS") return r.cfg.poller_sleep_ms;
  if (k == "GRPC_RDMA_MAX_SGE") return r.cfg.max_sge;
  return -1;
}


extern "C" void* b200_mem_alloc_device(size_t bytes) {
  if (!ensure_init()) return nullptr;
  void* p = nullptr;
  cudaSetDevice(R().dev);
  if (!CU_OK(cudaMalloc(&p, bytes ? bytes : 1))) return nullptr;
  reg_add(p, bytes ? bytes : 1, 2);
  return p;
}
extern "C" void b200_mem_free_device(void* p) {
  if (!p) return;
  reg_del(p);
  rt_free(p, 0);
}
extern "C" void* b200_mem_alloc_host(size_t bytes) {
  if (!ensure_init()) return nullptr;
  void* p = nullptr;
  cudaSetDevice(R().dev);
  if (!CU_OK(cudaHostAlloc(&p, bytes ? bytes : 1, cudaHostAllocMapped | cudaHostAllocPortable))) return nullptr;
  reg_add(p, bytes ? bytes : 1, 1);
  return p;
}
extern "C" void b200_mem_free_host(void* p) {
  if (!p) return;
  reg_del(p);
  rt_free(p, 1);
}
extern "C" int b200_mem_register_host(void* p, size_t bytes) {
  if (!ensure_init()) return -1;
  if (!CU_OK(cudaHostRegister(p, bytes, cudaHostRegisterMapped | cudaHostRegisterPortable))) return -1;
  reg_add(p, bytes, 1);
  return 0;
}
extern "C" int b200_mem_unregister_host(void* p) {
  reg_del(p);
  return CU_OK(cudaHostUnregister(p)) ? 0 : -1;
}
extern "C" int b200_memcpy(void* dst, const void* src, size_t bytes, int dir, void* stream) {
  if (!ensure_init()) return -1;
  cudaMemcpyKind k = dir == 0 ? cudaMemcpyHostToDevice : dir == 1 ? cudaMemcpyDeviceToHost : cudaMemcpyDeviceToDevice;
  cudaStream_t s = stream ? (cudaStream_t)stream : R().stream;
  return CU_OK(cudaMemcpyAsync(dst, src, bytes, k, s)) ? 0 : -1;
}
extern "C" int b200_stream_sync(void* stream) {
  if (!ensure_init()) return -1;
  cudaStream_t s = stream ? (cudaStream_t)stream : R().stream;
  return CU_OK(cudaStreamSynchronize(s)) ? 0 : -1;
}


extern "C" b200_pair* b200_pool_take(const char* id) {
  if (!ensure_init()) return nullptr;
  Runtime& r = R();
  std::lock_guard<std::mutex> lk(r.mu);
  b200_pair* p = nullptr;
  if (!r.pool.empty()) {
    p = r.pool.front();
    r.pool.pop();
  } else {
    if (r.free_slots.empty()) {
      set_err("b200_pool_take: connection table full");
      return nullptr;
    }
    p = new b200_pair();
    p->slot = r.free_slots.back();
    r.free_slots.pop_back();
    p->mirror = &r.h_mirrors[p->slot];
    p->wakeup_fd = eventfd(0, EFD_NONBLOCK | EFD_CLOEXEC);
    r.all_pairs.push_back(p);
  }
  p->id = id ? id : "";
  if (!p->id.empty()) r.id_pair[p->id] = p;
  return p;
}

extern "C" void b200_pool_putback(b200_pair* p) {
  if (!p) return;
  Runtime& r = R();
  std::lock_guard<std::mutex> lk(r.mu);
  auto it = r.id_pair.find(p->id);
  if (it != r.id_pair.end() && it->second == p) r.id_pair.erase(it);
  r.pool.push(p);
}

extern "C" b200_pair* b200_pool_get(const char* id) {
  Runtime& r = R();
  std::lock_guard<std::mutex> lk(r.mu);
  auto it = r.id_pair.find(id ? id : "");
  return it == r.id_pair.end() ? nullptr : it->second;
}

extern "C" void b200_pair_init(b200_pair* p) {
  if (!p || !ensure_init()) return;
  Runtime& r = R();
  std::lock_guard<std::mutex> lk(r.mu);
  if (!(p->status == B200_UNINITIALIZED || p->status == B200_ERROR || p->status == B200_DISCONNECTED)) return;
  cudaSetDevice(r.dev);
  const uint64_t cap = r.cfg.ring_bytes;
  if (!is_pow2(cap) || cap <= kReserved) {
    p->error = "ring buffer size must be a power of two > 24";
    set_err(p->error);
    p->status = B200_ERROR;
    return;
  }
  if (p->ring && p->cap != cap) {
    rt_free(p->ring, 0);
    p->ring = nullptr;
  }
  if (!p->ring) {
    if (!CU_OK(cudaMalloc(&p->ring, cap))) {
      p->error = t_err;
      p->status = B200_ERROR;
      return;
    }
  }
  p->cap = cap;
  PairDev hd;
  memset(&hd, 0, sizeof(hd));
  hd.ring = p->ring;
  hd.cap = cap;
  hd.mirror = p->mirror;
  hd.status = B200_INITIALIZED;
  hd.max_sge = (uint32_t)r.cfg.max_sge;
  hd.peer_slot = -1;
  p->max_sge = r.cfg.max_sge;
  p->svc_delivered = 0;
  p->retire_pending = false;
  p->peer_dead = false;
  p->peer_pid = 0;
  memset(p->mirror, 0, sizeof(PairMirror));
  bool ok = CU_OK(cudaMemsetAsync(p->ring, 0, cap, r.stream)) &&
            CU_OK(cudaMemcpyAsync(&r.d_pairs[p->slot], &hd, sizeof(hd), cudaMemcpyHostToDevice, r.stream)) &&
            CU_OK(cudaStreamSynchronize(r.stream));
  if (!ok) {
    p->error = t_err;
    p->status = B200_ERROR;
    return;
  }
  if (r.svc_running.load()) {
    const PairSvc fresh{0, ~0ull};
    memset((void*)&r.svc_erec[p->slot], 0, sizeof(EagerRec));
    cudaMemcpyAsync(&r.d_svc_psvc[p->slot], &fresh, sizeof(fresh), cudaMemcpyHostToDevice, r.stream);
    if ((uint32_t)p->slot + 1 > r.svc_hi_slot) {
      r.svc_hi_slot = (uint32_t)p->slot + 1;
      cudaMemcpyAsync(&r.d_svc_ps->hi_slot, &r.svc_hi_slot, 4, cudaMemcpyHostToDevice, r.stream);
    }
    cudaStreamSynchronize(r.stream);
    r.svc_gen++;
  }
  if (p->self.qpn) r.by_qpn.erase(p->self.qpn);
  memset(&p->self, 0, sizeof(p->self));
  p->self.lid = 0xB200;
  p->self.qpn = r.next_qpn++;
  p->self.psn = (uint32_t)rand() & 0xffffff;
  memcpy(p->self.gid, &r.cookie, 4);
  memcpy(p->self.gid + 4, &r.dev, 4);
  memcpy(p->self.gid + 8, &p->slot, 4);
  p->self.tag = B200_PAIR_TAG_POLLABLE;
  p->self.ring_buffer_size = cap;
  r.by_qpn[p->self.qpn] = p;
  p->peer_local = nullptr;
  p->remote = false;
  if (r.ipc_wire) {
    WireDesc d{};
    d.magic = kWireMagic;
    d.psn = p->self.psn;
    d.dev = r.dev;
    d.slot = p->slot;
    d.cap = cap;
    d.pid = (int32_t)getpid();
    d.pairs = r.pairs_handle;
    if (CU_OK(cudaIpcGetMemHandle(&d.ring, p->ring))) {
      p->wire_file = wire_path(r.cookie, p->self.qpn);
      const std::string tmp = p->wire_file + ".tmp";
      int fd = open(tmp.c_str(), O_CREAT | O_TRUNC | O_WRONLY, 0600);
      if (fd >= 0) {
        const bool okw = write(fd, &d, sizeof d) == (ssize_t)sizeof d;
        close(fd);
        if (okw) rename(tmp.c_str(), p->wire_file.c_str());
      }
    }
  }
  p->error.clear();
  eventfd_t junk;
  (void)eventfd_read(p->wakeup_fd, &junk);
  p->status = B200_INITIALIZED;
}

extern "C" size_t b200_pair_self_address(b200_pair* p, void* out48) {
  if (!p || !out48) return 0;
  memcpy(out48, &p->self, sizeof(AddrBlob));
  return sizeof(AddrBlob);
}

extern "C" int b200_pair_connect(b200_pair* p, const void* peer48, size_t n) {
  if (!p || !ensure_init()) return 0;
  Runtime& r = R();
  std::lock_guard<std::mutex> lk(r.mu);
  if (p->status != B200_INITIALIZED) return 0;
  if (n != sizeof(AddrBlob)) {
    p->error = "peer address blob has the wrong size";
    set_err(p->error);
    return 0;
  }
  memcpy(&p->peer, peer48, sizeof(AddrBlob));
  if (p->peer.tag != p->self.tag) {
    p->error = "peer pair tag mismatch";
    set_err(p->error);
    return 0;
  }
  if (p->peer.ring_buffer_size != p->self.ring_buffer_size) {
    p->error = "peer ring buffer size mismatch";
    set_err(p->error);
    return 0;
  }
  uint32_t cookie;
  memcpy(&cookie, p->peer.gid, 4);
  if (cookie != r.cookie) {
    WireDesc d{};
// ... 303 lines not shown
  r.launches += 3;
  r.svc_running = true;
  return 0;
}

extern "C" int b200_service_running(void) { return R().svc_running.load() ? R().svc_workers : 0; }

template <class Fill>
static bool svc_try_post(Runtime& r, int q, Fill fill, uint64_t* ticket) {
  Runtime::OwnerQ& Q = r.svc_q[q];
  std::lock_guard<std::mutex> lk(Q.mu);
  const uint64_t t = Q.next;
  const size_t e = (size_t)q * kOwnQ + t % kOwnQ;
  if (t >= kOwnQ && r.svc_consumed[e].load(std::memory_order_acquire) != (uint32_t)(t - kOwnQ + 1)) return false;
  Q.next = t + 1;
  SvcCmd* c = &r.svc_cmds[e];
  c->nreal = 0;
  fill(c, r.svc_slices + e * kSvcSliceArea);
  c->op = (c->op & 0xffu) | ((r.svc_gen.load(std::memory_order_acquire) & 0xffffffu) << 8);
  std::atomic_thread_fence(std::memory_order_release);
  *(volatile uint32_t*)&c->stamp2 = (uint32_t)(t + 1);
  *(volatile uint32_t*)&c->stamp = (uint32_t)(t + 1);
  *ticket = t;
  return true;
}
template <class Fill>
static uint64_t svc_post(Runtime& r, int q, Fill fill) {
  uint64_t t = 0;
  while (!svc_try_post(r, q, fill, &t)) {
#if defined(__x86_64__)
    __builtin_ia32_pause();
#endif
  }
  return t;
}

static bool svc_wait(Runtime& r, int q, uint64_t t, uint64_t* bytes, uint64_t* calls) {
  const size_t e = (size_t)q * kOwnQ + t % kOwnQ;
  volatile SvcDone* d = &r.svc_done[e];
  const uint32_t want = (uint32_t)(t + 1);
  uint32_t spins = 0;
  std::chrono::steady_clock::time_point t0;
  while (d->seq != want) {
    if ((int32_t)(d->seq - want) > 0) return true;
#if defined(__x86_64__)
    __builtin_ia32_pause();
#endif
    if ((++spins & 0xfffff) == 0) {
      if (spins == 0x100000) t0 = std::chrono::steady_clock::now();
      else if (std::chrono::steady_clock::now() - t0 > std::chrono::seconds(30)) {
        set_err("b200 service: command timed out");
        return false;
      }
    }
  }
  std::atomic_thread_fence(std::memory_order_acquire);
  if (bytes) *bytes = d->bytes;
  if (calls) *calls = d->calls;
  r.svc_consumed[e].store(want, std::memory_order_release);
  r.svc_ops++;
  return true;
}

static int owner_of(const Runtime& r, const b200_pair* p);
static int32_t slot_word(const b200_pair* p) {
  return (int32_t)((uint32_t)p->slot | (p->peer_local ? ((uint32_t)p->peer_local->slot + 1) << 16 : 0));
}
static void drain_retire(b200_pair* p) {
  Runtime& r = R();
  if (p->retire_owed.load(std::memory_order_acquire) && r.svc_running.load()) {
    const int q = owner_of(r, p);
    bool posted = false;
    const uint64_t t = svc_post(r, q, [&](SvcCmd* c, SliceDev*) {
      const uint32_t owed = p->retire_owed.exchange(0, std::memory_order_acq_rel);
      c->op = owed ? kSvcRetire : kSvcNop;
      c->slot = slot_word(p);
      c->flags = B200_BATCH_ONE_CALL;
      c->ptr = 0;
      c->n = owed;
      c->byte_idx = 0;
      posted = owed != 0;
    });
    (void)posted;
    svc_wait(r, q, t, nullptr, nullptr);
  }
}

extern "C" void b200_service_stop(void) {
  Runtime& r = R();
  if (!r.inited || !r.svc_running.load()) return;
  cudaSetDevice(r.dev);
  for (b200_pair* p : r.all_pairs) drain_retire(p);
  for (int q = 0; q < r.svc_nowners; q++) {
    const uint64_t t = svc_post(r, q, [&](SvcCmd* c, SliceDev*) { c->op = kSvcStop; });
    svc_wait(r, q, t, nullptr, nullptr);
  }
  uint32_t one = 1;
  cudaMemcpyAsync(&r.d_svc_ps->stop, &one, 4, cudaMemcpyHostToDevice, r.stream);
  cudaStreamSynchronize(r.stream);
  cudaStreamSynchronize(r.svc_stream);
  cudaStreamSynchronize(r.svc_stream_big);
  cudaStreamSynchronize(r.svc_stream_poll);
  r.svc_running = false;
  delete[] r.svc_q;
  r.svc_q = nullptr;
  delete[] r.svc_consumed;
  r.svc_consumed = nullptr;
  {
    std::lock_guard<std::mutex> lk(r.scan_mu);
    ReadyEntry* ring = r.svc_ready;
    r.svc_ready = nullptr;
    cudaFreeHost(ring);
  }
  cudaFreeHost(r.svc_cmds);
  cudaFreeHost(r.svc_done);
  cudaFreeHost(r.svc_slices);
  cudaFreeHost(r.svc_erec);
  cudaFreeHost(r.svc_eslots);
  cudaFreeHost(r.svc_host_scans);
  cudaFree(r.d_svc_ps);
  cudaFree(r.d_svc_last_ev);
  cudaFree(r.d_svc_boxes);
  cudaFree(r.d_svc_psvc);
  r.svc_cmds = nullptr;
  r.svc_done = nullptr;
  r.svc_slices = nullptr;
  r.svc_erec = nullptr;
  r.svc_eslots = nullptr;
  r.svc_host_scans = nullptr;
  r.d_svc_ps = nullptr;
  r.d_svc_last_ev = nullptr;
  r.d_svc_boxes = nullptr;
  r.d_svc_psvc = nullptr;
  r.svc_workers = 0;
  r.svc_nowners = 0;
  std::vector<std::pair<void*, int>> dead;
  {
    std::lock_guard<std::mutex> lk(r.grave_mu);
    dead.swap(r.graveyard);
  }
  for (auto& d : dead) {
    if (d.second) cudaFreeHost(d.first);
    else cudaFree(d.first);
  }
}

extern "C" void b200_service_stats(uint64_t out[4]) {
  Runtime& r = R();
  out[0] = r.svc_ops.load();
  out[1] = r.svc_ready_seen.load();
  out[2] = r.svc_ready_overflows.load();
  out[3] = r.svc_host_scans ? *(volatile uint32_t*)r.svc_host_scans : 0;
}
extern "C" uint64_t b200_service_eager_hits(void) { return R().svc_eager_hits.load(); }
extern "C" int b200_debug_service_trace(unsigned long long* out16) { return svc_trace_read(out16); }

static bool svc_fill_send(b200_pair* p, SvcCmd* c, SliceDev* area, const b200_slice* slices, size_t n, size_t byte_idx,
                          uint32_t flags, uint64_t* bounce_cursor = nullptr, uint8_t* own_bounce = nullptr,
                          uint64_t own_bounce_cap = 0) {
  const bool one_call = !(flags & B200_BATCH_UNTIL_BLOCKED);
  size_t look = n;
  if (one_call && look > (size_t)p->max_sge) look = (size_t)p->max_sge;
  if (look > kSvcSliceArea - 1) look = kSvcSliceArea - 1;
  TlsBounce own;
  own.tx = own_bounce;
  own.tx_cap = own_bounce_cap;
  uint64_t zero = 0;
  if (own_bounce && !bounce_cursor) bounce_cursor = &zero;
  TlsBounce& tb = own_bounce ? own : tls_bounce();
  uint64_t bounce_off = bounce_cursor ? *bounce_cursor : 0;
  for (size_t i = 0; i < look; i++) {
    const uint64_t len = slices[i].len;
    if (!len || mem_kind(slices[i].ptr) != 0) continue;
    const uint64_t skip = i == 0 ? byte_idx : 0;
    uint64_t take = len - skip;
    if (one_call && take > p->cap / 2) take = p->cap / 2;
    if (bounce_off + take > tb.tx_cap) {
      if (bounce_cursor == nullptr && bounce_off == 0) {
        if (!ensure_bounce(&tb.tx, &tb.tx_cap, (one_call ? p->cap : take) + 16 * (kMaxSgeLimit + 4))) return false;
      } else if (!one_call) {
        look = i;
        break;
      }
    }
    bounce_off += (take + 15) & ~15ull;
  }
  bounce_off = bounce_cursor ? *bounce_cursor : 0;
  uint64_t rest = 0;
  for (size_t i = look; i < n; i++) rest += slices[i].len;
  const size_t nsl = look + (rest ? 1 : 0);
  SliceDev* out = nsl <= kSvcInline ? c->inl : area;
  for (size_t i = 0; i < look; i++) {
    const uint8_t* ptr = (const uint8_t*)slices[i].ptr;
    const uint64_t len = slices[i].len;
    if (len && mem_kind(ptr) == 0) {
      const uint64_t skip = i == 0 ? byte_idx : 0;
      uint64_t take = len - skip;
      if (one_call && take > p->cap / 2) take = p->cap / 2;
      if (bounce_off + take > tb.tx_cap) take = tb.tx_cap - bounce_off;
      memcpy(tb.tx + bounce_off, ptr + skip, take);
      out[i].ptr = tb.tx + bounce_off - skip;
      bounce_off += (take + 15) & ~15ull;
    } else {
      out[i].ptr = ptr;
    }
    out[i].len = len;
  }
  if (bounce_cursor) *bounce_cursor = bounce_off;
  if (rest) {
    out[look].ptr = nullptr;
    out[look].len = rest;
  }
  c->op = kSvcSend;
  c->slot = slot_word(p);
  c->flags = flags;
  c->ptr = (uint64_t)(uintptr_t)area;
  c->n = nsl;
  c->nreal = (uint32_t)look;
  c->byte_idx = byte_idx;
  return true;
}

static uint64_t svc_send(Runtime& r, b200_pair* p, const b200_slice* slices, size_t n, size_t byte_idx) {
  const int q = owner_of(r, p);
  bool ok = true;
  const uint64_t t = svc_post(r, q, [&](SvcCmd* c, SliceDev* area) {
    const uint32_t owed = p->retire_owed.exchange(0, std::memory_order_acq_rel);
    ok = svc_fill_send(p, c, area, slices, n, byte_idx, B200_BATCH_ONE_CALL | (owed << 16));
    if (!ok) {
      c->op = owed ? kSvcRetire : kSvcNop;
      c->slot = slot_word(p);
      c->flags = B200_BATCH_ONE_CALL;
      c->n = owed;
    }
  });
  uint64_t bytes = 0;
  if (!svc_wait(r, q, t, &bytes, nullptr) || !ok) {
    p->error = t_err;
    p->status = B200_ERROR;
    return 0;
  }
  return bytes;
}

static uint64_t eager_checksum(const uint8_t* slot, uint32_t size, uint64_t at) {
  uint64_t cs = eager_mix(at * 31 + size);
  const uint32_t words = (size + 7) >> 3;
  for (uint32_t j = 0; j < words; j++) {
    uint64_t w = *(const volatile uint64_t*)(slot + 8ull * j);
    const uint32_t rem = size - 8 * j;
    if (rem < 8) w &= (1ull << (8 * rem)) - 1;
    cs ^= eager_word(w, j);
  }
  return cs;
}

static uint64_t svc_recv(Runtime& r, b200_pair* p, void* dst, uint64_t cap) {
  const int q = owner_of(r, p);
  const int kind = mem_kind3(dst);
  if (r.svc_erec && kind != 2 && !p->remote) {
    volatile EagerRec* rec = &r.svc_erec[p->slot];
    const uint8_t* slot = r.svc_eslots + (size_t)p->slot * kEagerMax;
    for (int attempt = 0; attempt < 4; attempt++) {
      const uint64_t at = rec->at;
      const uint32_t size = rec->size;
      if (rec->magic != kEagerMagic || at != p->svc_delivered || size == 0 || size > kEagerMax || size > cap) break;
      const uint64_t cs = rec->csum;
      memcpy(dst, slot, size);
      if (eager_checksum((const uint8_t*)dst, size, at) != cs) continue;
      p->svc_delivered += size;
      p->retire_owed.store(size, std::memory_order_release);
      r.svc_eager_hits++;
      return size;
    }
  }
  uint8_t* kdst = (uint8_t*)dst;
  uint64_t kcap = cap;
  TlsBounce& tb = tls_bounce();
  if (kind == 0) {
    if (kcap > p->cap) kcap = p->cap;
    if (!ensure_bounce(&tb.rx, &tb.rx_cap, p->cap)) return 0;
    kdst = tb.rx;
  }
  const uint64_t t = svc_post(r, q, [&](SvcCmd* c, SliceDev*) {
    c->op = kSvcRecv;
    c->slot = slot_word(p);
    c->flags = B200_BATCH_ONE_CALL;
    c->ptr = (uint64_t)(uintptr_t)kdst;
    c->n = kcap;
    c->byte_idx = 0;
  });
  uint64_t bytes = 0;
  if (!svc_wait(r, q, t, &bytes, nullptr)) {
    p->error = t_err;
    p->status = B200_ERROR;
    return 0;
  }
  p->svc_delivered += bytes;
  if (kind == 0 && bytes) memcpy(dst, tb.rx, bytes);
  return bytes;
}


static bool ensure_bounce(uint8_t** buf, uint64_t* cap, uint64_t need) {
  if (*cap >= need) return true;
  if (*buf) rt_free(*buf, 1);
  *buf = nullptr;
  *cap = 0;
  if (!CU_OK(cudaHostAlloc((void**)buf, need, cudaHostAllocMapped | cudaHostAllocPortable))) return false;
  *cap = need;
  return true;
}

static bool send_is_a_no_op(const b200_pair* p) {
  volatile PairMirror* m = p->mirror;
  if (!m->partial_write) return false;
  const uint64_t fr = free_size(p->cap, m->credit_head, m->remote_tail);
  const uint64_t lim = p->cap / 2 < fr ? p->cap / 2 : fr;
  return calc_writable(lim) == 0;
}

extern "C" uint64_t b200_pair_send(b200_pair* p, const b200_slice* slices, size_t n, size_t byte_idx) {
  if (!p || !ensure_init()) return 0;
  Runtime& r = R();
  if (p->peer_dead.load()) return 0;
  if (p->status == B200_CONNECTED && n) {
    if (p->peer_local) drain_retire(p->peer_local);
    refresh_remote(p);
    if (send_is_a_no_op(p)) return 0;
  }
  if (r.svc_running.load()) {
    if (p->status != B200_CONNECTED || n == 0) return 0;
    if (((volatile PairMirror*)p->mirror)->peer_exit == 1) return 0;
    return svc_send(r, p, slices, n, byte_idx);
  }
  std::lock_guard<std::mutex> lk(r.mu);
  if (p->status != B200_CONNECTED || n == 0) return 0;
  if (((volatile PairMirror*)p->mirror)->peer_exit == 1) return 0;
  cudaSetDevice(r.dev);
  const size_t look = n < (size_t)p->max_sge ? n : (size_t)p->max_sge;
  uint64_t rest = 0;
  for (size_t i = look; i < n; i++) rest += slices[i].len;
  uint64_t bounce_off = 0;
  for (size_t i = 0; i < look; i++) {
    const uint8_t* ptr = (const uint8_t*)slices[i].ptr;
    uint64_t len = slices[i].len;
    if (len && mem_kind(ptr) == 0) {
      const uint64_t skip = i == 0 ? byte_idx : 0;
      const uint64_t useful = len - skip;
      const uint64_t limit = p->cap / 2;
      uint64_t take = useful < limit ? useful : limit;
      if (!ensure_bounce(&r.bounce_tx, &r.bounce_tx_cap, p->cap + 16 * (kMaxSgeLimit + 4))) return 0;
      if (bounce_off + take > r.bounce_tx_cap) take = r.bounce_tx_cap - bounce_off;
      memcpy(r.bounce_tx + bounce_off, ptr + skip, take);
      r.h_slices[i].ptr = r.bounce_tx + bounce_off - skip;
      bounce_off += (take + 15) & ~15ull;
    } else {
      r.h_slices[i].ptr = ptr;
    }
    r.h_slices[i].len = len;
  }
  size_t nsl = look;
  if (rest) {
    r.h_slices[nsl].ptr = nullptr;
    r.h_slices[nsl].len = rest;
    nsl++;
  }
  r.h_sop->slot = p->slot;
  r.h_sop->flags = B200_BATCH_ONE_CALL;
  r.h_sop->slices = r.h_slices;
  r.h_sop->nslices = nsl;
  r.h_sop->nreal = look;
  r.h_sop->byte_idx = byte_idx;
  r.h_res->bytes = 0;
  r.h_res->calls = 0;
  launch_send(r.d_pairs, r.h_sop, r.h_res, 1, r.stream);
  r.launches++;
  if (!CU_OK(cudaGetLastError()) || !CU_OK(cudaStreamSynchronize(r.stream))) {
    p->error = t_err;
    p->status = B200_ERROR;
    return 0;
  }
  return r.h_res->bytes;
}

extern "C" uint64_t b200_pair_recv(b200_pair* p, void* dst, uint64_t cap) {
  if (!p || !ensure_init()) return 0;
  Runtime& r = R();
  drain_retire(p);
  if (p->status == B200_CONNECTED && !p->remote && ((volatile PairMirror*)p->mirror)->has_message == 0) return 0;
  if (r.svc_running.load()) {
    if (p->status != B200_CONNECTED || cap == 0) return 0;
    return svc_recv(r, p, dst, cap);
  }
  std::lock_guard<std::mutex> lk(r.mu);
  if (p->status != B200_CONNECTED || cap == 0) return 0;
  cudaSetDevice(r.dev);
  const bool bounce = mem_kind(dst) == 0;
  uint8_t* kdst = (uint8_t*)dst;
  uint64_t kcap = cap;
  if (bounce) {
    if (kcap > p->cap) kcap = p->cap;
    if (!ensure_bounce(&r.bounce_rx, &r.bounce_rx_cap, p->cap)) return 0;
    kdst = r.bounce_rx;
  }
  r.h_rop->slot = p->slot;
  r.h_rop->flags = B200_BATCH_ONE_CALL;
  r.h_rop->dst = kdst;
  r.h_rop->cap = kcap;
  r.h_res->bytes = 0;
  r.h_res->calls = 0;
  launch_recv(r.d_pairs, r.h_rop, r.h_res, 1, r.stream);
  r.launches++;
  if (!CU_OK(cudaGetLastError()) || !CU_OK(cudaStreamSynchronize(r.stream))) {
    p->error = t_err;
    p->status = B200_ERROR;
    return 0;
  }
  const uint64_t got = r.h_res->bytes;
  if (bounce && got) memcpy(dst, r.bounce_rx, got);
  return got;
}


static int mem_class(const void* p) {
  cudaPointerAttributes a;
  if (cudaPointerGetAttributes(&a, p) != cudaSuccess) {
    cudaGetLastError();
    return 0;
  }
  if (a.type == cudaMemoryTypeHost) return 1;
  if (a.type == cudaMemoryTypeUnregistered) return 0;
  return 2;
}

static int lane_of(const b200_pair* p) {
  static const int nl = [] { long v = env_long("B200_LANES", 8); return (int)(v < 1 ? 1 : v > kLanes ? kLanes : v); }();
  static const int shift = (int)env_long("B200_LANE_SHIFT", 1);
  int key = p->slot;
  if (p->peer_local && p->peer_local->slot < key) key = p->peer_local->slot;
  return (key >> shift) % nl;
}

constexpr size_t kDmaAlign = 4096;

static size_t stage_place(size_t& cursor, const void* host_ptr, size_t bytes) {
  size_t off = ((cursor + kDmaAlign - 1) & ~(kDmaAlign - 1)) + ((uintptr_t)host_ptr & (kDmaAlign - 1));
  cursor = off + bytes;
  return off;
}

constexpr size_t kHostDmaAlign = 256;
static void push_h2d(std::vector<CopyRun>& out, uint8_t* stage, const uint8_t* src, size_t bytes) {
  if (!bytes) return;
  size_t lead = (uintptr_t)src & (kHostDmaAlign - 1);
  if (lead) {
    Runtime& r = R();
    std::lock_guard<std::mutex> lk(r.reg_mu);
    auto it = r.reg_ranges.upper_bound((uintptr_t)src);
    if (it == r.reg_ranges.begin()) {
      lead = 0;
    } else {
      --it;
      if ((uintptr_t)src >= it->first + it->second.first || (uintptr_t)src - lead < it->first) lead = 0;
    }
  }
  out.push_back({stage - lead, src - lead, lead + bytes});
}

static b200_batch* prepare_common(int kind, const void* ops_v, size_t nops, int flags) {
  if (!ensure_init()) return nullptr;
  Runtime& r = R();
  cudaSetDevice(r.dev);
  b200_batch* b = new b200_batch();
  b->kind = kind;
  b->nops = (int)nops;
  b->flags = flags;
  const b200_send_op* sops = (const b200_send_op*)ops_v;
  const b200_recv_op* rops = (const b200_recv_op*)ops_v;
  bool ok = true;
  int cls = -1;
  for (size_t i = 0; ok && i < nops; i++) {
    const b200_pair* pr = kind == 0 ? sops[i].pair : rops[i].pair;
    if (!pr) {
      set_err("batch: null pair");
      ok = false;
      break;
    }
    const void* probe = nullptr;
    if (kind == 0) {
      for (size_t j = 0; j < sops[i].nslices && !probe; j++)
        if (sops[i].slices[j].len) probe = sops[i].slices[j].ptr;
    } else if (rops[i].cap) {
      probe = rops[i].dst;
    }
    if (!probe) continue;
    const int c = mem_class(probe);
    if (c == 0) {
      set_err("batch: slices / destinations must be GPU-addressable (device memory, b200_mem_alloc_host or "
              "b200_mem_register_host); unregistered host memory is only accepted by b200_pair_send/recv");
      ok = false;
    } else if (cls >= 0 && c != cls) {
      set_err("batch: host and device buffers cannot be mixed in one batch");
      ok = false;
    }
    cls = c;
  }
  b->staged = ok && cls == 1 && !(flags & B200_BATCH_ZEROCOPY);
  b->perm.resize(nops);
  if (ok && b->staged) {
    int k = 0;
    for (int L = 0; L < kLanes; L++) {
      b->lanes[L].first_op = k;
      for (size_t i = 0; i < nops; i++)
        if (lane_of(kind == 0 ? sops[i].pair : rops[i].pair) == L) b->perm[k++] = (int)i;
      b->lanes[L].nops = k - b->lanes[L].first_op;
    }
  } else {
    for (size_t i = 0; i < nops; i++) b->perm[i] = (int)i;
  }
  const uint32_t kflags = (uint32_t)(flags & (B200_BATCH_UNTIL_BLOCKED | B200_BATCH_CONCURRENT));
  if (ok && kind == 0) {
    size_t total_slices = 0;
    for (size_t i = 0; i < nops; i++) total_slices += sops[i].nslices;
    std::vector<SendOpDev> h(nops ? nops : 1);
    std::vector<SliceDev> hs(total_slices ? total_slices : 1);
    std::vector<size_t> stage_off(total_slices ? total_slices : 1, 0);
    ok = CU_OK(cudaMalloc(&b->d_slices, sizeof(SliceDev) * hs.size())) &&
         CU_OK(cudaMalloc(&b->d_ops, sizeof(SendOpDev) * (nops ? nops : 1)));
    size_t off = 0, cursor = 0;
    struct Run { int lane; const uint8_t* src; size_t bytes, stage; };
    std::vector<Run> runs;
    for (size_t k = 0; ok && k < nops; k++) {
      const b200_send_op& o = sops[b->perm[k]];
      h[k].slot = o.pair->slot;
      h[k].flags = kflags;
      h[k].slices = b->d_slices + off;
      h[k].nslices = o.nslices;
      h[k].nreal = o.nslices;
      h[k].byte_idx = o.byte_idx;
      const int L = b->staged ? lane_of(o.pair) : 0;
      const uint8_t* run_end = nullptr;
      for (size_t j = 0; j < o.nslices; j++) {
        const uint8_t* ptr = (const uint8_t*)o.slices[j].ptr;
        const uint64_t len = o.slices[j].len;
        hs[off + j].ptr = ptr;
        hs[off + j].len = len;
        if (b->staged && len) {
          if (runs.empty() || runs.back().lane != L || ptr != run_end) {
            Run nr = {L, ptr, 0, 0};
            nr.stage = stage_place(cursor, ptr, 0);
            runs.push_back(nr);
          }
          stage_off[off + j] = runs.back().stage + runs.back().bytes;
          runs.back().bytes += len;
          cursor = runs.back().stage + runs.back().bytes;
          run_end = ptr + len;
        }
      }
      off += o.nslices;
    }
    if (ok && b->staged) {
      ok = CU_OK(cudaMalloc(&b->d_stage, cursor + kDmaAlign));
      for (size_t q = 0; ok && q < total_slices; q++)
        if (hs[q].len) hs[q].ptr = b->d_stage + stage_off[q];
      for (const Run& rn : runs) push_h2d(b->lanes[rn.lane].copies, b->d_stage + rn.stage, rn.src, rn.bytes);
    }
    ok = ok && CU_OK(cudaMemcpy(b->d_slices, hs.data(), sizeof(SliceDev) * hs.size(), cudaMemcpyHostToDevice)) &&
         CU_OK(cudaMemcpy(b->d_ops, h.data(), sizeof(SendOpDev) * (nops ? nops : 1), cudaMemcpyHostToDevice));
  } else if (ok) {
    std::vector<RecvOpDev> h(nops ? nops : 1);
    ok = CU_OK(cudaMalloc(&b->d_ops, sizeof(RecvOpDev) * (nops ? nops : 1)));
    size_t cursor = 0;
    std::vector<size_t> place(nops ? nops : 1, 0);
    for (size_t k = 0; k < nops; k++) {
      const b200_recv_op& o = rops[b->perm[k]];
      h[k].slot = o.pair->slot;
      h[k].flags = kflags;
      h[k].dst = (uint8_t*)o.dst;
      h[k].cap = o.cap;
      b->pairs.push_back(o.pair);
      if (b->staged && o.cap) place[k] = stage_place(cursor, o.dst, o.cap);
    }
    if (ok && b->staged) {
      ok = CU_OK(cudaMalloc(&b->d_stage, cursor + kDmaAlign)) && CU_OK(cudaMemset(b->d_stage, 0, cursor + kDmaAlign));
      for (size_t k = 0; ok && k < nops; k++) {
        const b200_recv_op& o = rops[b->perm[k]];
        if (!o.cap) continue;
        h[k].dst = b->d_stage + place[k];
        b->lanes[lane_of(o.pair)].copies.push_back({o.dst, b->d_stage + place[k], (size_t)o.cap});
      }
    }
    ok = ok && CU_OK(cudaMemcpy(b->d_ops, h.data(), sizeof(RecvOpDev) * (nops ? nops : 1), cudaMemcpyHostToDevice));
  }
  ok = ok && CU_OK(cudaMalloc(&b->d_results, sizeof(OpResult) * (nops ? nops : 1))) &&
       CU_OK(cudaHostAlloc(&b->h_results, sizeof(OpResult) * (nops ? nops : 1), cudaHostAllocPortable));
  if (!ok) {
    b200_batch_destroy(b);
    return nullptr;
  }
  return b;
}

extern "C" b200_batch* b200_batch_prepare_send(const b200_send_op* ops, size_t nops, int flags) {
  return prepare_common(0, ops, nops, flags);
}
extern "C" b200_batch* b200_batch_prepare_recv(const b200_recv_op* ops, size_t nops, int flags) {
  return prepare_common(1, ops, nops, flags);
}

extern "C" int b200_lanes_fork(void* stream) {
  if (!ensure_init() || !stream) return -1;
  Runtime& r = R();
  if (!CU_OK(cudaEventRecord(r.fork_event, (cudaStream_t)stream))) return -1;
  for (int L = 0; L < kLanes; L++)
    if (!CU_OK(cudaStreamWaitEvent(r.lane_up[L], r.fork_event, 0)) ||
        !CU_OK(cudaStreamWaitEvent(r.lane_down[L], r.fork_event, 0)))
      return -1;
  return 0;
}

extern "C" int b200_lanes_join(void* stream) {
  if (!ensure_init()) return -1;
  Runtime& r = R();
  for (int L = 0; L < kLanes; L++) {
    if (stream) {
      if (!CU_OK(cudaEventRecord(r.join_up[L], r.lane_up[L])) ||
          !CU_OK(cudaEventRecord(r.join_down[L], r.lane_down[L])) ||
          !CU_OK(cudaStreamWaitEvent((cudaStream_t)stream, r.join_up[L], 0)) ||
          !CU_OK(cudaStreamWaitEvent((cudaStream_t)stream, r.join_down[L], 0)))
        return -1;
    } else if (!CU_OK(cudaStreamSynchronize(r.lane_up[L])) || !CU_OK(cudaStreamSynchronize(r.lane_down[L]))) {
      return -1;
    }
  }
  return 0;
}

extern "C" int b200_batch_launch(b200_batch* b, void* stream) {
  if (!b) return -1;
  Runtime& r = R();
  if (b->nops == 0) return 0;
  if (r.svc_running.load()) r.svc_gen++;
  if (b->kind == 1 && r.svc_running.load()) {
    for (b200_pair* p : b->pairs) {
      drain_retire(p);
      ((volatile EagerRec*)&r.svc_erec[p->slot])->magic = 0;
      p->svc_delivered += 1ull << 40;
    }
  }
  if (!b->staged) {
    cudaStream_t s = stream ? (cudaStream_t)stream : r.stream;
    if (b->kind == 0) launch_send(r.d_pairs, (const SendOpDev*)b->d_ops, b->d_results, b->nops, s);
    else launch_recv(r.d_pairs, (const RecvOpDev*)b->d_ops, b->d_results, b->nops, s);
    r.launches++;
    return CU_OK(cudaGetLastError()) ? 0 : -1;
  }
  if (stream && b200_lanes_fork(stream) != 0) return -1;
  for (int L = 0; L < kLanes; L++) {
    LanePlan& lp = b->lanes[L];
    if (lp.nops == 0) continue;
    if (b->kind == 0) {
      cudaStream_t s = r.lane_up[L];
      for (const CopyRun& c : lp.copies)
        if (!CU_OK(cudaMemcpyAsync(c.dst, c.src, c.bytes, cudaMemcpyHostToDevice, s))) return -1;
      if (!CU_OK(cudaStreamWaitEvent(s, r.recv_done[L], 0))) return -1;
      launch_send(r.d_pairs, (const SendOpDev*)b->d_ops + lp.first_op, b->d_results + lp.first_op, lp.nops, s);
      if (!CU_OK(cudaEventRecord(r.send_done[L], s))) return -1;
    } else {
      cudaStream_t s = r.lane_down[L];
      if (!CU_OK(cudaStreamWaitEvent(s, r.send_done[L], 0))) return -1;
      launch_recv(r.d_pairs, (const RecvOpDev*)b->d_ops + lp.first_op, b->d_results + lp.first_op, lp.nops, s);
      if (!CU_OK(cudaEventRecord(r.recv_done[L], s))) return -1;
      for (const CopyRun& c : lp.copies)
        if (!CU_OK(cudaMemcpyAsync(c.dst, c.src, c.bytes, cudaMemcpyDeviceToHost, s))) return -1;
    }
    r.launches++;
    if (!CU_OK(cudaGetLastError())) return -1;
  }
  if (stream && b200_lanes_join(stream) != 0) return -1;
  return 0;
}

extern "C" int b200_batch_results(b200_batch* b, uint64_t* out, void* stream) {
  if (!b) return -1;
  Runtime& r = R();
  if (b->nops == 0) return 0;
  cudaStream_t s = stream ? (cudaStream_t)stream : r.stream;
  if (b->staged) {
    for (int L = 0; L < kLanes; L++)
      if (b->lanes[L].nops &&
          (!CU_OK(cudaStreamSynchronize(r.lane_up[L])) || !CU_OK(cudaStreamSynchronize(r.lane_down[L]))))
        return -1;
  }
  if (!CU_OK(cudaMemcpyAsync(b->h_results, b->d_results, sizeof(OpResult) * b->nops, cudaMemcpyDeviceToHost, s)) ||
      !CU_OK(cudaStreamSynchronize(s)))
    return -1;
  if (out)
    for (int k = 0; k < b->nops; k++) out[b->perm[k]] = b->h_results[k].bytes;
  return 0;
}

extern "C" int b200_batch_calls(b200_batch* b, uint64_t* out) {
  if (!b || !out) return -1;
  for (int k = 0; k < b->nops; k++) out[b->perm[k]] = b->h_results[k].calls;
  return 0;
}

extern "C" void b200_batch_destroy(b200_batch* b) {
  if (!b) return;
  rt_free(b->d_ops, 0);
  rt_free(b->d_slices, 0);
  rt_free(b->d_results, 0);
  rt_free(b->d_stage, 0);
  rt_free(b->h_results, 1);
  delete b;
}

static int run_unprepared(int kind, const void* ops, size_t nops, int flags, uint64_t* out, void* stream) {
  b200_batch* b = prepare_common(kind, ops, nops, flags);
  if (!b) return -1;
  int rc = b200_batch_launch(b, stream);
  if (rc == 0) rc = b200_batch_results(b, out, stream);
  b200_batch_destroy(b);
  return rc;
}

extern "C" int b200_pairs_send(const b200_send_op* ops, size_t nops, int flags, uint64_t* accepted, void* stream) {
  return run_unprepared(0, ops, nops, flags, accepted, stream);
}
extern "C" int b200_pairs_recv(const b200_recv_op* ops, size_t nops, int flags, uint64_t* delivered, void* stream) {
  return run_unprepared(1, ops, nops, flags, delivered, stream);
}

extern "C" int b200_pairs_submit(const b200_send_op* sops, size_t ns, uint64_t* accepted, const b200_recv_op* rops,
                                 size_t nr, uint64_t* delivered, int flags) {
  if (!ensure_init()) return -1;
  Runtime& r = R();
  if (!r.svc_running.load()) {
    int rc = 0;
    if (ns) rc = b200_pairs_send(sops, ns, flags, accepted, nullptr);
    if (rc == 0 && nr) rc = b200_pairs_recv(rops, nr, flags, delivered, nullptr);
    return rc;
  }
  struct Ticket {
    int q;
    uint64_t t;
    bool posted;
  };
  static thread_local std::vector<Ticket> st, rt;
  st.assign(ns, Ticket{0, 0, false});
  rt.assign(nr, Ticket{0, 0, false});
  uint64_t need = 0;
  for (size_t i = 0; i < ns; i++)
    for (size_t j = 0; j < sops[i].nslices && j < kSvcSliceArea; j++)
      if (sops[i].slices[j].len && mem_kind(sops[i].slices[j].ptr) == 0) need += (sops[i].slices[j].len + 15) & ~15ull;
  TlsBounce& tb = tls_bounce();
  const uint64_t kMaxBounce = 1ull << 30;
  if (need && !ensure_bounce(&tb.tx, &tb.tx_cap, need < kMaxBounce ? need : kMaxBounce)) return -1;
  uint64_t cursor = 0;
  const uint32_t fl = (uint32_t)(flags & (B200_BATCH_UNTIL_BLOCKED));
  int rc = 0;
  static const uint64_t kStageMin = (uint64_t)env_long("B200_SUBMIT_STAGE_MIN", 1l << 40);
  static thread_local std::vector<uint8_t*> rstage;
  rstage.assign(nr, nullptr);
  {
    uint64_t want = 0;
    for (size_t i = 0; i < nr; i++)
      if (rops[i].cap >= kStageMin && mem_kind3(rops[i].dst) == 1) want += (rops[i].cap + 255) & ~255ull;
    if (want) {
      cudaSetDevice(r.dev);
      if (want > tb.dstage_cap) {
        if (tb.dstage) rt_free(tb.dstage, 0);
        tb.dstage = nullptr;
        tb.dstage_cap = 0;
        if (CU_OK(cudaMalloc(&tb.dstage, want))) tb.dstage_cap = want;
      }
      if (!tb.copy_stream && !CU_OK(cudaStreamCreateWithFlags(&tb.copy_stream, cudaStreamNonBlocking))) tb.copy_stream = nullptr;
      if (tb.dstage && tb.copy_stream) {
        uint64_t off = 0;
        for (size_t i = 0; i < nr; i++)
          if (rops[i].cap >= kStageMin && mem_kind3(rops[i].dst) == 1) {
            rstage[i] = tb.dstage + off;
            off += (rops[i].cap + 255) & ~255ull;
          }
      }
    }
  }
  bool copies = false;
  auto harvest = [&]() {
    for (size_t i = 0; i < ns; i++) {
      if (!st[i].posted) continue;
      st[i].posted = false;
      uint64_t bytes = 0;
      if (!svc_wait(r, st[i].q, st[i].t, &bytes, nullptr)) rc = -1;
      if (accepted) accepted[i] = bytes;
    }
    for (size_t i = 0; i < nr; i++) {
      if (!rt[i].posted) continue;
      rt[i].posted = false;
      uint64_t bytes = 0;
      if (!svc_wait(r, rt[i].q, rt[i].t, &bytes, nullptr)) rc = -1;
      rops[i].pair->svc_delivered += bytes;
      if (delivered) delivered[i] = bytes;
      if (rstage[i] && bytes) {
        if (!CU_OK(cudaMemcpyAsync(rops[i].dst, rstage[i], bytes, cudaMemcpyDeviceToHost, tb.copy_stream))) rc = -1;
        copies = true;
      }
    }
  };
  for (size_t i = 0; i < ns; i++) {
    b200_pair* p = sops[i].pair;
    if (accepted) accepted[i] = 0;
    if (!p || p->status != B200_CONNECTED || sops[i].nslices == 0) continue;
    if (((volatile PairMirror*)p->mirror)->peer_exit == 1) continue;
    if (p->peer_local && p->peer_local->retire_owed.load(std::memory_order_acquire)) {
      harvest();
      drain_retire(p->peer_local);
    }
    if (send_is_a_no_op(p)) continue;
    const int q = owner_of(r, p);
    bool ok = true;
    auto fill = [&](SvcCmd* c, SliceDev* area) {
      const uint32_t owed = p->retire_owed.exchange(0, std::memory_order_acq_rel);
      ok = svc_fill_send(p, c, area, sops[i].slices, sops[i].nslices, sops[i].byte_idx, fl | (owed << 16), &cursor);
      if (!ok) {
        c->op = owed ? kSvcRetire : kSvcNop;
        c->slot = slot_word(p);
        c->flags = B200_BATCH_ONE_CALL;
        c->n = owed;
      }
    };
    while (!svc_try_post(r, q, fill, &st[i].t)) harvest();
    st[i].q = q;
    st[i].posted = true;
  }
  for (size_t i = 0; i < nr; i++) {
    b200_pair* p = rops[i].pair;
    if (delivered) delivered[i] = 0;
    if (!p || p->status != B200_CONNECTED || rops[i].cap == 0) continue;
    if (p->retire_owed.load(std::memory_order_acquire)) {
      harvest();
      drain_retire(p);
    }
    if (!p->remote && ((volatile PairMirror*)p->mirror)->has_message == 0) continue;
    if (mem_kind(rops[i].dst) == 0) {
      set_err("b200_pairs_submit: destinations must be GPU-addressable (b200_mem_alloc_host / register_host / device)");
      rc = -1;
      continue;
    }
    const int q = owner_of(r, p);
    auto fill = [&](SvcCmd* c, SliceDev*) {
      c->op = kSvcRecv;
      c->slot = slot_word(p);
      c->flags = fl;
      c->ptr = (uint64_t)(uintptr_t)(rstage[i] ? rstage[i] : (uint8_t*)rops[i].dst);
      c->n = rops[i].cap;
      c->byte_idx = 0;
    };
    while (!svc_try_post(r, q, fill, &rt[i].t)) harvest();
    rt[i].q = q;
    rt[i].posted = true;
  }
  harvest();
  if (copies && !CU_OK(cudaStreamSynchronize(tb.copy_stream))) rc = -1;
  return rc;
}


struct b200_async {
  int kind = 0;
  b200_pair* p = nullptr;
  int q = 0;
  uint64_t t = 0;
  int state = 0;
  uint64_t bytes = 0;
  uint8_t* stage = nullptr;
  int stage_cls = -1;
  uint8_t* hstage = nullptr;
  int hstage_cls = -1;
  void* dst = nullptr;
  cudaEvent_t ev = nullptr;
};

namespace {
struct AsyncPool {
  std::mutex mu;
  std::vector<uint8_t*> free_stage[32], free_hstage[32];
  std::vector<b200_async*> free_ops;
  cudaStream_t copy[4] = {nullptr, nullptr, nullptr, nullptr};
  std::atomic<uint32_t> rr{0};
};
AsyncPool& AP() {
  static AsyncPool a;
  return a;
}
b200_async* async_get() {
  AsyncPool& a = AP();
  {
    std::lock_guard<std::mutex> lk(a.mu);
    if (!a.free_ops.empty()) {
      b200_async* o = a.free_ops.back();
      a.free_ops.pop_back();
      return o;
    }
  }
  b200_async* o = new b200_async();
  cudaEventCreateWithFlags(&o->ev, cudaEventDisableTiming);
  return o;
}
void async_put(b200_async* o) {
  AsyncPool& a = AP();
  std::lock_guard<std::mutex> lk(a.mu);
  if (o->stage) a.free_stage[o->stage_cls].push_back(o->stage);
  if (o->hstage) a.free_hstage[o->hstage_cls].push_back(o->hstage);
  o->stage = o->hstage = nullptr;
  o->stage_cls = o->hstage_cls = -1;
  o->state = 0;
  a.free_ops.push_back(o);
}
uint8_t* stage_get(uint64_t bytes, int* cls) {
  int c = 16;
  while ((1ull << c) < bytes) c++;
  *cls = c;
  AsyncPool& a = AP();
  {
    std::lock_guard<std::mutex> lk(a.mu);
    if (!a.free_stage[c].empty()) {
      uint8_t* p = a.free_stage[c].back();
      a.free_stage[c].pop_back();
      return p;
    }
  }
  uint8_t* p = nullptr;
  cudaSetDevice(R().dev);
  if (cudaMalloc(&p, 1ull << c) != cudaSuccess) {
    cudaGetLastError();
    return nullptr;
  }
  return p;
}
}

extern "C" b200_async* b200_pair_post_send(b200_pair* p, const b200_slice* slices, size_t n, size_t byte_idx, int flags,
                                           int* again) {
  if (again) *again = 0;
  Runtime& r = R();
  if (!p || !r.svc_running.load()) {
    set_err("b200_pair_post_send: the service is not running");
    return nullptr;
  }
  b200_async* o = async_get();
  o->kind = 0;
  o->p = p;
  o->bytes = 0;
  o->state = 2;
  if (p->status != B200_CONNECTED || n == 0 || ((volatile PairMirror*)p->mirror)->peer_exit == 1) return o;
  if (p->peer_local) drain_retire(p->peer_local);
  if (send_is_a_no_op(p)) return o;
  const int q = owner_of(r, p);
  bool ok = true;
  uint64_t t = 0;
  {
    uint64_t need = 0;
    for (size_t i = 0; i < n && i < kSvcSliceArea; i++)
      if (slices[i].len && mem_kind(slices[i].ptr) == 0) need += (slices[i].len + 15) & ~15ull;
    if (need) {
      int c = 12;
      while ((1ull << c) < need && c < 28) c++;
      AsyncPool& a = AP();
      {
        std::lock_guard<std::mutex> lk(a.mu);
        if (!a.free_hstage[c].empty()) {
          o->hstage = a.free_hstage[c].back();
          a.free_hstage[c].pop_back();
        }
      }
      if (!o->hstage && cudaHostAlloc((void**)&o->hstage, 1ull << c, cudaHostAllocMapped | cudaHostAllocPortable) != cudaSuccess) {
        cudaGetLastError();
        o->hstage = nullptr;
      }
      o->hstage_cls = c;
      if (!o->hstage) {
        set_err("b200_pair_post_send: pinned staging allocation failed");
        async_put(o);
        return nullptr;
      }
    }
  }
  auto fill = [&](SvcCmd* c, SliceDev* area) {
    const uint32_t owed = p->retire_owed.exchange(0, std::memory_order_acq_rel);
    ok = svc_fill_send(p, c, area, slices, n, byte_idx, (uint32_t)(flags & B200_BATCH_UNTIL_BLOCKED) | (owed << 16), nullptr,
                       o->hstage, o->hstage ? 1ull << o->hstage_cls : 0);
    if (!ok) {
      c->op = owed ? kSvcRetire : kSvcNop;
      c->slot = slot_word(p);
      c->flags = B200_BATCH_ONE_CALL;
      c->n = owed;
    }
  };
  if (!svc_try_post(r, q, fill, &t)) {
    async_put(o);
    if (again) *again = 1;
    return nullptr;
  }
  o->q = q;
  o->t = t;
  o->state = 0;
  return o;
}

extern "C" b200_async* b200_pair_post_recv(b200_pair* p, void* dst, uint64_t cap, int flags, int* again) {
  if (again) *again = 0;
  Runtime& r = R();
  if (!p || !r.svc_running.load()) {
    set_err("b200_pair_post_recv: the service is not running");
    return nullptr;
// ... 226 lines not shown
```

Baseline: 1086.

## Spread send/recv ops across a grid-wide work-stealing mover pool

Replaces the one-CTA-per-op send/recv kernels with a persistent grid sized by total bytes and occupancy. Producers publish chunk work items into per-op global-memory rings, and mover warps in any CTA claim and copy them, stealing from other rings when their own is empty. The goal is to let large ops such as 4 MiB payloads use more SMs than the op count allows. The cost is global-memory queue traffic, atomics and release/acquire fences, plus a work-area allocation and memset per batch.

```diff
diff --git a/grpc-rdma_b200/csrc/b200_dev.cuh b/grpc-rdma_b200/csrc/b200_dev.cuh
--- a/grpc-rdma_b200/csrc/b200_dev.cuh
+++ b/grpc-rdma_b200/csrc/b200_dev.cuh
@@ -1,4 +1,5 @@
 #pragma once
+#include <stddef.h>
 #include <stdint.h>
 
 #if defined(__CUDACC__)
@@ -180,8 +181,13 @@
   int nowners, nbig;
 };
 
-void launch_send(PairDev* pairs, const SendOpDev* ops, OpResult* results, int nops, void* stream);
-void launch_recv(PairDev* pairs, const RecvOpDev* ops, OpResult* results, int nops, void* stream);
+int grid_limit();
+int grid_for(int nops, uint64_t bytes);
+size_t grid_work_bytes(int grid);
+void launch_send(PairDev* pairs, const SendOpDev* ops, OpResult* results, int nops, int grid, void* work,
+                 void* stream);
+void launch_recv(PairDev* pairs, const RecvOpDev* ops, OpResult* results, int nops, int grid, void* work,
+                 void* stream);
 void launch_poll_scan(PairDev* pairs, const int32_t* slots, uint32_t* events, uint32_t* ready_count,
                       int32_t* ready_slots, int n, void* stream);
 
diff --git a/grpc-rdma_b200/csrc/b200_kernels.cu b/grpc-rdma_b200/csrc/b200_kernels.cu
--- a/grpc-rdma_b200/csrc/b200_kernels.cu
+++ b/grpc-rdma_b200/csrc/b200_kernels.cu
@@ -237,6 +237,21 @@
   __threadfence_block();
   *(volatile uint32_t*)&slot->ready = id + 1;
 }
+
+struct SmemQueue {
+  static constexpr uint32_t kSize = kQI;
+  WorkItem* q;
+  PipeCtl* ctl;
+  __device__ __forceinline__ void publish(uint32_t id, uint64_t a, uint64_t b, uint64_t c, uint32_t n) const {
+    publish_item(q, id, a, b, c, n);
+  }
+  __device__ __forceinline__ void finish(uint32_t total_items, uint32_t op_done) const {
+    ctl->total_items = total_items;
+    ctl->op_done = op_done;
+    __threadfence_block();
+    *(volatile uint32_t*)&ctl->seg_done = 1;
+  }
+};
 
 __device__ __forceinline__ void movers_init(uint64_t* bars, uint32_t tid) {
   if (tid < kMovers * kDepth) mbar_init(&bars[tid], 1);
@@ -318,8 +333,9 @@
   uint32_t first_item[kMaxSgeLimit + 1];
 };
 
+template <class Queue>
 __device__ __noinline__ void send_produce_segment(const SendOpDev& op, const PairDev* P, uint8_t* ring,
-                                                  SendPlanState& S, SendCallScratch& CS, WorkItem* q, PipeCtl* ctl,
+                                                  SendPlanState& S, SendCallScratch& CS, const Queue& Q,
                                                   uint32_t* foot8, uint32_t* nfoot_out, uint32_t lane) {
   const uint64_t cap = S.cap, mask = cap - 1;
   uint32_t base_item = 0, nfoot = 0;
@@ -412,14 +428,14 @@
     __syncwarp();
     nfoot += nframes;
     const unsigned big = __ballot_sync(0xffffffffu, items > 8);
-    if (!big && nitems <= kQI) {
+    if (!big && nitems <= Queue::kSize) {
       const uint32_t first = items_incl - items;
       for (uint32_t t = 0; t < items; t++) {
         const uint64_t c0 = (uint64_t)t * kChunk;
         uint64_t n = p - c0;
         if (n > kChunk) n = kChunk;
-        publish_item(q, base_item + first + t, reinterpret_cast<uint64_t>(ptr + c0), (foff + 8 + c0) & mask,
-                     c0 == 0 ? p : 0, (uint32_t)n);
+        Q.publish(base_item + first + t, reinterpret_cast<uint64_t>(ptr + c0), (foff + 8 + c0) & mask,
+                  c0 == 0 ? p : 0, (uint32_t)n);
       }
     } else
     for (uint32_t it = lane; it < nitems; it += 32) {
@@ -429,8 +445,8 @@
       const uint64_t flen = CS.len[f];
       uint64_t n = flen - c0;
       if (n > kChunk) n = kChunk;
-      publish_item(q, base_item + it, reinterpret_cast<uint64_t>(CS.src[f] + c0), (CS.off[f] + 8 + c0) & mask,
-                   c0 == 0 ? flen : 0, (uint32_t)n);
+      Q.publish(base_item + it, reinterpret_cast<uint64_t>(CS.src[f] + c0), (CS.off[f] + 8 + c0) & mask,
+                c0 == 0 ? flen : 0, (uint32_t)n);
     }
     __syncwarp();
     base_item += nitems;
@@ -442,10 +458,7 @@
   }
   if (lane == 0) {
     *nfoot_out = nfoot;
-    ctl->total_items = base_item;
-    ctl->op_done = op_done ? 1u : 0u;
-    __threadfence_block();
-    *(volatile uint32_t*)&ctl->seg_done = 1;
+    Q.finish(base_item, op_done ? 1u : 0u);
   }
   __syncwarp();
 }
@@ -469,6 +482,47 @@
     if (n > seg1) smem_to_global(ring, stage, pre + (uint32_t)seg1, n - (uint32_t)seg1, lane);
   }
 };
+
+__device__ __forceinline__ uint32_t send_plan_init(const PairDev* P, const SendOpDev& op, SendPlanState& PS) {
+  PS.rt = *(volatile uint64_t*)&P->remote_tail;
+  PS.cap = *(volatile uint64_t*)&P->cap;
+  PS.staging = PS.cap / 2;
+  PS.max_sge = *(volatile uint32_t*)&P->max_sge;
+  PS.cur = 0;
+  PS.bidx = op.byte_idx;
+  PS.written_total = 0;
+  PS.ncalls = 0;
+  PS.partial = *(volatile uint32_t*)&P->partial_write;
+  PS.last_rh = ~0ull;
+  return *(volatile uint32_t*)&P->status;
+}
+
+__device__ __forceinline__ void send_finish(PairDev* __restrict__ pairs, PairDev* P, const SendOpDev& op,
+                                            const SendPlanState& PS, OpResult* result) {
+  P->remote_tail = PS.rt;
+  P->partial_write = PS.partial;
+  result->bytes = PS.written_total;
+  result->calls = PS.ncalls;
+  const bool conc = (op.flags & kFlagConcurrent) != 0;
+  mirror_lock(P, conc);
+  publish_mirror_tx(VL(P->mirror), P);
+  mirror_unlock(P, conc);
+  const int peer_slot = VL(P->peer_slot);
+  if (peer_slot >= 0 && PS.written_total) {
+    PairDev* Q = &pairs[peer_slot];
+    PairMirror* qm = VL(Q->mirror);
+    if (qm) {
+      uint32_t hm;
+      uint64_t rd;
+      mirror_lock(Q, conc);
+      rx_probe<false>(VL(Q->ring), VL(Q->cap), *(volatile uint64_t*)&Q->head, *(volatile uint64_t*)&Q->remain, hm, rd);
+      volatile PairMirror* vm = qm;
+      vm->has_message = hm;
+      vm->readable = rd;
+      mirror_unlock(Q, conc);
+    }
+  }
+}
 
 struct PipeSmem {
   WorkItem q[kQI];
@@ -493,17 +547,7 @@
   if (tid < kQI) q[tid].ready = 0;
   if (tid == 0) {
     s_total = 0;
-    s_status = *(volatile uint32_t*)&P->status;
-    PS.rt = *(volatile uint64_t*)&P->remote_tail;
-    PS.cap = *(volatile uint64_t*)&P->cap;
-    PS.staging = PS.cap / 2;
-    PS.max_sge = *(volatile uint32_t*)&P->max_sge;
-    PS.cur = 0;
-    PS.bidx = op.byte_idx;
-    PS.written_total = 0;
-    PS.ncalls = 0;
-    PS.partial = *(volatile uint32_t*)&P->partial_write;
-    PS.last_rh = ~0ull;
+    s_status = send_plan_init(P, op, PS);
   }
   __syncthreads();
   {
@@ -535,7 +579,7 @@
     }
     __syncthreads();
     if (warp == 0) {
-      send_produce_segment(op, P, ring, PS, CS, q, &ctl, foot8, &s_nfoot, lane);
+      send_produce_segment(op, P, ring, PS, CS, SmemQueue{q, &ctl}, foot8, &s_nfoot, lane);
     } else {
       const SendMove mv{ring, cap, mask};
       mover_run(mv, q, &ctl, stage_mem + (warp - 1) * (kDepth * kStageBytes), &bars[(warp - 1) * kDepth], phase_bits, lane);
@@ -550,42 +594,9 @@
     __syncthreads();
     if (done) break;
   }
-  if (tid == 0) {
-    P->remote_tail = PS.rt;
-    P->partial_write = PS.partial;
-    result->bytes = PS.written_total;
-    result->calls = PS.ncalls;
-    const bool conc = (op.flags & kFlagConcurrent) != 0;
-    mirror_lock(P, conc);
-    publish_mirror_tx(VL(P->mirror), P);
-    mirror_unlock(P, conc);
-    const int peer_slot = VL(P->peer_slot);
-    if (peer_slot >= 0 && PS.written_total) {
-      PairDev* Q = &pairs[peer_slot];
-      PairMirror* qm = VL(Q->mirror);
-      if (qm) {
-        uint32_t hm;
-        uint64_t rd;
-        mirror_lock(Q, conc);
-        rx_probe<false>(VL(Q->ring), VL(Q->cap), *(volatile uint64_t*)&Q->head, *(volatile uint64_t*)&Q->remain, hm, rd);
-        volatile PairMirror* vm = qm;
-        vm->has_message = hm;
-        vm->readable = rd;
-        mirror_unlock(Q, conc);
-      }
-    }
-  }
-}
-
-__global__ void __launch_bounds__(kThreads, 2)
-k_send(PairDev* __restrict__ pairs, const SendOpDev* __restrict__ ops, OpResult* __restrict__ results) {
-  extern __shared__ __align__(128) uint8_t stage_mem[];
-  __shared__ PipeSmem pipe;
-  movers_init(pipe.bars, threadIdx.x);
-  uint32_t phase_bits = 0;
-  const SendOpDev op = ops[blockIdx.x];
-  send_body(pairs, op, &results[blockIdx.x], pipe, stage_mem, phase_bits);
-}
+  if (tid == 0) send_finish(pairs, P, op, PS, result);
+}
+
 
 
 struct ScoutState {
@@ -594,8 +605,9 @@
   uint32_t credit_flag;
 };
 
+template <class Queue>
 __device__ __noinline__ void recv_produce_segment(const RecvOpDev& op, const uint8_t* ring, uint64_t cap,
-                                                  ScoutState& SS, WorkItem* q, PipeCtl* ctl, uint32_t lane) {
+                                                  ScoutState& SS, const Queue& Q, uint32_t lane) {
   const uint64_t mask = cap - 1;
   uint64_t head = SS.head, mh = SS.mh, remain = SS.remain, acc = SS.acc, cap_left = SS.cap_left;
   uint64_t delivered = SS.delivered, ncalls = SS.ncalls;
@@ -772,7 +784,7 @@
         const bool tail_item = m <= kChunk;
         if (m > kChunk) m = kChunk;
         const uint64_t z = (c0 == 0 ? f_zh : 0u) | ((uint64_t)(tail_item ? f_zt : 0u) << 16);
-        publish_item(q, base_item + it, (f_src + c0) & mask, f_dst + c0, z, (uint32_t)m);
+        Q.publish(base_item + it, (f_src + c0) & mask, f_dst + c0, z, (uint32_t)m);
       }
     }
     __syncwarp();
@@ -824,10 +836,7 @@
     SS.ncalls = ncalls;
     SS.credit_flag = credit;
     SS.credit_val = credit_val;
-    ctl->total_items = base_item;
-    ctl->op_done = last;
-    __threadfence_block();
-    *(volatile uint32_t*)&ctl->seg_done = 1;
+    Q.finish(base_item, last);
   }
   __syncwarp();
 }
@@ -868,6 +877,48 @@
   }
 };
 
+__device__ __forceinline__ uint32_t recv_scout_init(const PairDev* P, const RecvOpDev& op, ScoutState& SS) {
+  SS.head = *(volatile uint64_t*)&P->head;
+  SS.mh = *(volatile uint64_t*)&P->moving_head;
+  SS.remain = *(volatile uint64_t*)&P->remain;
+  SS.acc = *(volatile uint64_t*)&P->acc;
+  SS.cap_left = op.cap;
+  SS.delivered = 0;
+  SS.ncalls = 0;
+  SS.credit_flag = 0;
+  return *(volatile uint32_t*)&P->status;
+}
+
+__device__ __forceinline__ void recv_credit(PairDev* __restrict__ pairs, PairDev* P, const RecvOpDev& op,
+                                            ScoutState& SS) {
+  const int peer_slot = VL(P->peer_slot);
+  const bool conc = (op.flags & kFlagConcurrent) != 0 && peer_slot >= 0;
+  PairDev* Q = conc ? &pairs[peer_slot] : nullptr;
+  if (conc) mirror_lock(Q, true);
+  st_release_v2u64(VL(P->peer_credit), SS.credit_val, 0);
+  PairMirror* pm = VL(P->peer_mirror);
+  if (pm) ((volatile PairMirror*)pm)->credit_head = SS.credit_val;
+  if (conc) mirror_unlock(Q, true);
+  SS.credit_flag = 0;
+}
+
+__device__ __forceinline__ void recv_finish(PairDev* P, const RecvOpDev& op, const ScoutState& SS,
+                                            const uint8_t* ring, uint64_t cap, OpResult* result) {
+  P->head = SS.head;
+  P->moving_head = SS.mh;
+  P->remain = SS.remain;
+  P->acc = SS.acc;
+  result->bytes = SS.delivered;
+  result->calls = SS.ncalls;
+  uint32_t hm;
+  uint64_t rd;
+  const bool conc = (op.flags & kFlagConcurrent) != 0;
+  mirror_lock(P, conc);
+  rx_probe<false>(ring, cap, SS.head, SS.remain, hm, rd);
+  publish_mirror_rx(VL(P->mirror), P, hm, rd);
+  mirror_unlock(P, conc);
+}
+
 __device__ __forceinline__ void recv_body(PairDev* __restrict__ pairs, const RecvOpDev& op, OpResult* result,
                                           PipeSmem& pipe, uint8_t* stage_mem, uint32_t& phase_bits) {
   WorkItem* q = pipe.q;
@@ -879,17 +930,7 @@
   const uint32_t tid = threadIdx.x, lane = tid & 31, warp = tid >> 5;
 
   if (tid < kQI) q[tid].ready = 0;
-  if (tid == 0) {
-    s_status = *(volatile uint32_t*)&P->status;
-    SS.head = *(volatile uint64_t*)&P->head;
-    SS.mh = *(volatile uint64_t*)&P->moving_head;
-    SS.remain = *(volatile uint64_t*)&P->remain;
-    SS.acc = *(volatile uint64_t*)&P->acc;
-    SS.cap_left = op.cap;
-    SS.delivered = 0;
-    SS.ncalls = 0;
-    SS.credit_flag = 0;
-  }
+  if (tid == 0) s_status = recv_scout_init(P, op, SS);
   __syncthreads();
   if (s_status != kStConnected) {
     if (tid == 0) {
@@ -910,7 +951,7 @@
     }
     __syncthreads();
     if (warp == 0) {
-      recv_produce_segment(op, ring, cap, SS, q, &ctl, lane);
+      recv_produce_segment(op, ring, cap, SS, SmemQueue{q, &ctl}, lane);
     } else {
       const RecvMove mv{ring, op.dst, cap, mask};
       mover_run(mv, q, &ctl, stage_mem + (warp - 1) * (kDepth * kStageBytes), &bars[(warp - 1) * kDepth], phase_bits, lane);
@@ -919,45 +960,339 @@
     if (credit) __threadfence_system();
     __syncthreads();
     const bool done = ctl.op_done != 0;
-    if (tid == 0 && credit) {
-      const int peer_slot = VL(P->peer_slot);
-      const bool conc = (op.flags & kFlagConcurrent) != 0 && peer_slot >= 0;
-      PairDev* Q = conc ? &pairs[peer_slot] : nullptr;
-      if (conc) mirror_lock(Q, true);
-      st_release_v2u64(VL(P->peer_credit), SS.credit_val, 0);
-      PairMirror* pm = VL(P->peer_mirror);
-      if (pm) ((volatile PairMirror*)pm)->credit_head = SS.credit_val;
-      if (conc) mirror_unlock(Q, true);
-      SS.credit_flag = 0;
-    }
+    if (tid == 0 && credit) recv_credit(pairs, P, op, SS);
     __syncthreads();
     if (done) break;
   }
+  if (tid == 0) recv_finish(P, op, SS, ring, cap, result);
+}
+
+
+
+constexpr uint32_t kGQ = 64;
+constexpr uint64_t kGridBytesPerCta = 1ull << 20;
+
+struct __align__(128) GridCtl {
+  uint32_t op_next;
+  uint32_t ops_done;
+  uint32_t exits;
+};
+struct __align__(128) GridRing {
+  uint32_t next;
+  uint32_t _p0[31];
+  uint32_t done;
+  uint32_t _p1[31];
+  uint8_t* ring;
+  uint8_t* dst;
+  uint64_t cap;
+  uint32_t sys;
+  uint32_t _p2[25];
+  WorkItem q[kGQ];
+};
+static_assert(sizeof(GridRing) == 3 * 128 + kGQ * sizeof(WorkItem), "GridRing layout");
+
+__device__ __forceinline__ uint32_t ld_volatile_u32(const void* p) {
+  uint32_t v;
+  asm volatile("ld.volatile.global.u32 %0, [%1];" : "=r"(v) : "l"(p) : "memory");
+  return v;
+}
+__device__ __forceinline__ uint32_t ld_acquire_gpu_u32(const void* p) {
+  uint32_t v;
+  asm volatile("ld.acquire.gpu.global.u32 %0, [%1];" : "=r"(v) : "l"(p) : "memory");
+  return v;
+}
+__device__ __forceinline__ void st_release_gpu_u32(void* p, uint32_t v) {
+  asm volatile("st.release.gpu.global.u32 [%0], %1;" ::"l"(p), "r"(v) : "memory");
+}
+
+struct GridQueue {
+  static constexpr uint32_t kSize = kGQ;
+  GridRing* r;
+  uint32_t base;
+  uint32_t* seg;
+  __device__ __forceinline__ void publish(uint32_t id, uint64_t a, uint64_t b, uint64_t c, uint32_t n) const {
+    id += base;
+    WorkItem* s = &r->q[id % kGQ];
+    while (ld_acquire_gpu_u32(&s->ready) != 0) __nanosleep(20);
+    s->a = a;
+    s->b = b;
+    s->c = c;
+    s->n = n;
+    st_release_gpu_u32(&s->ready, id + 1);
+  }
+  __device__ __forceinline__ void finish(uint32_t total_items, uint32_t op_done) const {
+    seg[0] = total_items;
+    seg[1] = op_done;
+  }
+};
+
+struct GridStage {
+  uint64_t a, b, c;
+  uint8_t* ring;
+  uint8_t* dst;
+  uint64_t cap;
+  uint32_t n, ridx, sys, _pad;
+};
+
+template <class Move> __device__ __forceinline__ Move grid_move(const GridStage& g);
+template <> __device__ __forceinline__ SendMove grid_move<SendMove>(const GridStage& g) {
+  return SendMove{g.ring, g.cap, g.cap - 1};
+}
+template <> __device__ __forceinline__ RecvMove grid_move<RecvMove>(const GridStage& g) {
+  return RecvMove{g.ring, g.dst, g.cap, g.cap - 1};
+}
+
+template <class Move>
+__device__ __forceinline__ uint32_t grid_claim(GridRing* rings, uint32_t ridx, uint32_t want, uint32_t tail,
+                                               GridStage* gs, uint8_t* stages, uint64_t* bars, uint32_t lane) {
+  GridRing* R = &rings[ridx];
+  uint32_t t = 0;
+  if (lane == 0) t = ld_volatile_u32(&R->next);
+  t = __shfl_sync(0xffffffffu, t, 0);
+  const bool pub = lane < want && ld_acquire_gpu_u32(&R->q[(t + lane) % kGQ].ready) == t + lane + 1;
+  const uint32_t k = __ffs(~__ballot_sync(0xffffffffu, pub)) - 1;
+  if (k == 0) return 0;
+  uint32_t won = 0;
+  if (lane == 0) won = atomicCAS(&R->next, t, t + k) == t;
+  if (!__shfl_sync(0xffffffffu, won, 0)) return 0;
+  if (lane < k) {
+    WorkItem* w = &R->q[(t + lane) % kGQ];
+    const uint32_t s = (tail + lane) % kDepth;
+    GridStage& g = gs[s];
+    g.a = VL(w->a);
+    g.b = VL(w->b);
+    g.c = VL(w->c);
+    g.n = VL(w->n);
+    g.ring = VL(R->ring);
+    g.dst = VL(R->dst);
+    g.cap = VL(R->cap);
+    g.sys = VL(R->sys);
+    g.ridx = ridx;
+    st_release_gpu_u32(&w->ready, 0);
+    grid_move<Move>(g).issue(g.a, g.n, stages + s * kStageBytes, &bars[s]);
+  }
+  __syncwarp();
+  return k;
+}
+
+template <class Move>
+__device__ __forceinline__ void grid_mover(GridCtl* gc, GridRing* rings, uint32_t grid, uint32_t nops, GridStage* gs,
+                                           uint8_t* stages, uint64_t* bars, uint32_t lane, uint32_t wid) {
+  const uint32_t own = blockIdx.x;
+  uint32_t head = 0, tail = 0, phase_bits = 0;
+  uint32_t pend_r = 0, pend_n = 0, pend_sys = 0;
+  uint32_t victim = own * 7 + wid * 37, idle = 0;
+  auto flush = [&]() {
+    if (pend_n == 0) return;
+    if (pend_sys) __threadfence_system();
+    else __threadfence();
+    __syncwarp();
+    if (lane == 0) atomicAdd(&rings[pend_r].done, pend_n);
+    pend_n = 0;
+    pend_sys = 0;
+  };
+  while (true) {
+    bool dry = false;
+    if (tail - head < (uint32_t)kDepth) {
+      const uint32_t want = kDepth - (tail - head);
+      uint32_t got = 0;
+      for (int tries = 0; tries < 4 && got == 0; tries++) {
+        got = grid_claim<Move>(rings, own, want, tail, gs, stages, bars, lane);
+        if (got == 0 && tries == 0) {
+          const uint32_t t = ld_volatile_u32(&rings[own].next);
+          const bool more = ld_volatile_u32(&rings[own].q[t % kGQ].ready) == t + 1;
+          if (!__shfl_sync(0xffffffffu, more, 0)) break;
+        }
+      }
+      for (uint32_t seen = 0; got == 0 && seen < grid; seen += 32) {
+        const uint32_t v = (victim + seen + lane) % grid;
+        bool has = false;
+        if (seen + lane < grid && v != own) {
+          const uint32_t t = ld_volatile_u32(&rings[v].next);
+          has = ld_volatile_u32(&rings[v].q[t % kGQ].ready) == t + 1;
+        }
+        const unsigned m = __ballot_sync(0xffffffffu, has);
+        if (m) {
+          const uint32_t vl = __ffs(m) - 1;
+          got = grid_claim<Move>(rings, __shfl_sync(0xffffffffu, v, vl), want, tail, gs, stages, bars, lane);
+          victim += seen + vl;
+        }
+      }
+      if (got == 0) victim += 32;
+      dry = got == 0;
+      tail += got;
+    }
+    if (head == tail) {
+      flush();
+      if (ld_volatile_u32(&gc->ops_done) >= nops) break;
+      __nanosleep(64u << (idle < 4 ? idle : 4));
+      idle++;
+      continue;
+    }
+    idle = 0;
+    const uint32_t s = head % kDepth;
+    const GridStage g = gs[s];
+    if (pend_n && g.ridx != pend_r) flush();
+    const uint32_t par = (phase_bits >> s) & 1u;
+    while (!mbar_try_wait(&bars[s], par)) {
+    }
+    phase_bits ^= 1u << s;
+    grid_move<Move>(g).process(g.a, g.b, g.c, g.n, stages + s * kStageBytes, lane);
+    __syncwarp();
+    pend_r = g.ridx;
+    pend_n++;
+    pend_sys |= g.sys;
+    head++;
+    if (dry) flush();
+  }
+}
+
+__device__ __forceinline__ void grid_wait_done(GridRing* R, uint32_t published, bool sys, uint32_t lane) {
+  if (lane == 0)
+    while (ld_volatile_u32(&R->done) != published) __nanosleep(32);
+  __syncwarp();
+  if (sys) __threadfence_system();
+  else __threadfence();
+}
+
+__device__ __forceinline__ void grid_set_context(GridRing* R, uint8_t* ring, uint8_t* dst, uint64_t cap, bool sys,
+                                                 uint32_t lane) {
+  if (lane == 0) {
+    VL(R->ring) = ring;
+    VL(R->dst) = dst;
+    VL(R->cap) = cap;
+    VL(R->sys) = sys ? 1u : 0u;
+    __threadfence();
+  }
+  __syncwarp();
+}
+
+__device__ __forceinline__ void send_op_grid(PairDev* __restrict__ pairs, const SendOpDev& op, OpResult* result,
+                                             GridRing* R, uint32_t& base, uint32_t lane) {
+  __shared__ SendPlanState PS;
+  __shared__ SendCallScratch CS;
+  __shared__ uint32_t foot8[kFootCap];
+  __shared__ uint32_t s_nfoot, s_status;
+  __shared__ uint32_t s_seg[2];
+  PairDev* P = &pairs[op.slot];
+  if (lane == 0) s_status = send_plan_init(P, op, PS);
+  unsigned long long total = 0;
+  for (uint64_t i = lane; i < op.nslices; i += 32) total += op.slices[i].len;
+  for (int o = 16; o > 0; o >>= 1) total += __shfl_xor_sync(0xffffffffu, total, o);
+  __syncwarp();
+  if (s_status != kStConnected) {
+    if (lane == 0) {
+      result->bytes = 0;
+      result->calls = 0;
+    }
+    return;
+  }
+  if (lane == 0) PS.total_left = total - op.byte_idx;
+  const uint64_t cap = VL(P->cap);
+  uint8_t* ring = VL(P->peer_ring);
+  const bool sys_scope = VL(P->wire) != 0;
+  grid_set_context(R, ring, nullptr, cap, sys_scope, lane);
+  while (true) {
+    send_produce_segment(op, P, ring, PS, CS, GridQueue{R, base, s_seg}, foot8, &s_nfoot, lane);
+    base += s_seg[0];
+    grid_wait_done(R, base, sys_scope, lane);
+    const uint32_t nfoot = s_nfoot;
+    for (uint32_t i = lane; i < nfoot; i += 32) *reinterpret_cast<uint64_t*>(ring + ((uint64_t)foot8[i] << 3)) = kFooter;
+    const bool done = s_seg[1] != 0;
+    __syncwarp();
+    if (done) break;
+  }
+  if (lane == 0) send_finish(pairs, P, op, PS, result);
+  __syncwarp();
+}
+
+__device__ __forceinline__ void recv_op_grid(PairDev* __restrict__ pairs, const RecvOpDev& op, OpResult* result,
+                                             GridRing* R, uint32_t& base, uint32_t lane) {
+  __shared__ ScoutState SS;
+  __shared__ uint32_t s_status;
+  __shared__ uint32_t s_seg[2];
+  PairDev* P = &pairs[op.slot];
+  if (lane == 0) s_status = recv_scout_init(P, op, SS);
+  __syncwarp();
+  if (s_status != kStConnected) {
+    if (lane == 0) {
+      result->bytes = 0;
+      result->calls = 0;
+    }
+    return;
+  }
+  uint8_t* ring = VL(P->ring);
+  const uint64_t cap = VL(P->cap);
+  const bool sys_scope = VL(P->wire) != 0;
+  grid_set_context(R, ring, op.dst, cap, sys_scope, lane);
+  while (true) {
+    recv_produce_segment(op, ring, cap, SS, GridQueue{R, base, s_seg}, lane);
+    base += s_seg[0];
+    grid_wait_done(R, base, sys_scope, lane);
+    if (SS.credit_flag) {
+      __threadfence_system();
+      __syncwarp();
+      if (lane == 0) recv_credit(pairs, P, op, SS);
+    }
+    const bool done = s_seg[1] != 0;
+    __syncwarp();
+    if (done) break;
+  }
+  if (lane == 0) recv_finish(P, op, SS, ring, cap, result);
+  __syncwarp();
+}
+
+template <class Op, class Move, void (*Body)(PairDev*, const Op&, OpResult*, GridRing*, uint32_t&, uint32_t)>
+__device__ __forceinline__ void grid_kernel(PairDev* pairs, const Op* ops, OpResult* results, uint32_t nops,
+                                            GridCtl* gc, GridRing* rings, uint8_t* stage_mem) {
+  __shared__ uint64_t bars[kMovers * kDepth];
+  __shared__ GridStage gs[kMovers][kDepth];
+  const uint32_t tid = threadIdx.x, lane = tid & 31, warp = tid >> 5;
+  GridRing* R = &rings[blockIdx.x];
+  movers_init(bars, tid);
   if (tid == 0) {
-    P->head = SS.head;
-    P->moving_head = SS.mh;
-    P->remain = SS.remain;
-    P->acc = SS.acc;
-    result->bytes = SS.delivered;
-    result->calls = SS.ncalls;
-    uint32_t hm;
-    uint64_t rd;
-    const bool conc = (op.flags & kFlagConcurrent) != 0;
-    mirror_lock(P, conc);
-    rx_probe<false>(ring, cap, SS.head, SS.remain, hm, rd);
-    publish_mirror_rx(VL(P->mirror), P, hm, rd);
-    mirror_unlock(P, conc);
+    VL(R->next) = 0;
+    VL(R->done) = 0;
+  }
+  __syncthreads();
+  if (warp == 0) {
+    uint32_t base = 0;
+    while (true) {
+      uint32_t k = 0;
+      if (lane == 0) k = atomicAdd(&gc->op_next, 1u);
+      k = __shfl_sync(0xffffffffu, k, 0);
+      if (k >= nops) break;
+      const Op op = ops[k];
+      Body(pairs, op, &results[k], R, base, lane);
+      if (lane == 0) {
+        __threadfence();
+        atomicAdd(&gc->ops_done, 1u);
+      }
+    }
+  } else {
+    grid_mover<Move>(gc, rings, gridDim.x, nops, gs[warp - 1], stage_mem + (warp - 1) * (kDepth * kStageBytes),
+                     &bars[(warp - 1) * kDepth], lane, warp);
+  }
+  __syncthreads();
+  if (tid == 0 && atomicAdd(&gc->exits, 1u) == gridDim.x - 1) {
+    VL(gc->op_next) = 0;
+    VL(gc->ops_done) = 0;
+    VL(gc->exits) = 0;
   }
 }
 
 __global__ void __launch_bounds__(kThreads, 2)
-k_recv(PairDev* __restrict__ pairs, const RecvOpDev* __restrict__ ops, OpResult* __restrict__ results) {
+k_send(PairDev* __restrict__ pairs, const SendOpDev* __restrict__ ops, OpResult* __restrict__ results, uint32_t nops,
+       GridCtl* gc, GridRing* rings) {
   extern __shared__ __align__(128) uint8_t stage_mem[];
-  __shared__ PipeSmem pipe;
-  movers_init(pipe.bars, threadIdx.x);
-  uint32_t phase_bits = 0;
-  const RecvOpDev op = ops[blockIdx.x];
-  recv_body(pairs, op, &results[blockIdx.x], pipe, stage_mem, phase_bits);
+  grid_kernel<SendOpDev, SendMove, send_op_grid>(pairs, ops, results, nops, gc, rings, stage_mem);
+}
+
+__global__ void __launch_bounds__(kThreads, 2)
+k_recv(PairDev* __restrict__ pairs, const RecvOpDev* __restrict__ ops, OpResult* __restrict__ results, uint32_t nops,
+       GridCtl* gc, GridRing* rings) {
+  extern __shared__ __align__(128) uint8_t stage_mem[];
+  grid_kernel<RecvOpDev, RecvMove, recv_op_grid>(pairs, ops, results, nops, gc, rings, stage_mem);
 }
 
 
@@ -1906,15 +2241,44 @@
 }
 
 
-void launch_send(PairDev* pairs, const SendOpDev* ops, OpResult* results, int nops, void* stream) {
+int grid_limit() {
+  static const int lim = [] {
+    ensure_kernel_attrs();
+    int dev = 0, sms = 0, ps = 0, pr = 0;
+    cudaGetDevice(&dev);
+    cudaDeviceGetAttribute(&sms, cudaDevAttrMultiProcessorCount, dev);
+    if (cudaOccupancyMaxActiveBlocksPerMultiprocessor(&ps, k_send, kThreads, kStageTotal) != cudaSuccess ||
+        cudaOccupancyMaxActiveBlocksPerMultiprocessor(&pr, k_recv, kThreads, kStageTotal) != cudaSuccess)
+      return 1;
+    const int per_sm = ps < pr ? ps : pr;
+    return per_sm * sms > 0 ? per_sm * sms : 1;
+  }();
+  return lim;
+}
+int grid_for(int nops, uint64_t bytes) {
+  uint64_t g = (bytes + kGridBytesPerCta - 1) / kGridBytesPerCta;
+  if (g < (uint64_t)nops) g = (uint64_t)nops;
+  const int lim = grid_limit();
+  if (g > (uint64_t)lim) g = (uint64_t)lim;
+  return g < 1 ? 1 : (int)g;
+}
+size_t grid_work_bytes(int grid) { return sizeof(GridCtl) + sizeof(GridRing) * (size_t)grid; }
+
+void launch_send(PairDev* pairs, const SendOpDev* ops, OpResult* results, int nops, int grid, void* work,
+                 void* stream) {
   if (nops <= 0) return;
   ensure_kernel_attrs();
-  k_send<<<nops, kThreads, kStageTotal, static_cast<cudaStream_t>(stream)>>>(pairs, ops, results);
-}
-void launch_recv(PairDev* pairs, const RecvOpDev* ops, OpResult* results, int nops, void* stream) {
+  GridCtl* gc = static_cast<GridCtl*>(work);
+  k_send<<<grid, kThreads, kStageTotal, static_cast<cudaStream_t>(stream)>>>(
+      pairs, ops, results, (uint32_t)nops, gc, reinterpret_cast<GridRing*>(gc + 1));
+}
+void launch_recv(PairDev* pairs, const RecvOpDev* ops, OpResult* results, int nops, int grid, void* work,
+                 void* stream) {
   if (nops <= 0) return;
   ensure_kernel_attrs();
-  k_recv<<<nops, kThreads, kStageTotal, static_cast<cudaStream_t>(stream)>>>(pairs, ops, results);
+  GridCtl* gc = static_cast<GridCtl*>(work);
+  k_recv<<<grid, kThreads, kStageTotal, static_cast<cudaStream_t>(stream)>>>(
+      pairs, ops, results, (uint32_t)nops, gc, reinterpret_cast<GridRing*>(gc + 1));
 }
 void launch_poll_scan(PairDev* pairs, const int32_t* slots, uint32_t* events, uint32_t* ready_count,
                       int32_t* ready_slots, int n, void* stream) {
diff --git a/grpc-rdma_b200/csrc/b200_runtime.cu b/grpc-rdma_b200/csrc/b200_runtime.cu
--- a/grpc-rdma_b200/csrc/b200_runtime.cu
+++ b/grpc-rdma_b200/csrc/b200_runtime.cu
@@ -97,6 +97,8 @@
 
 struct LanePlan {
   int first_op = 0, nops = 0;
+  int grid = 0;
+  size_t grid_off = 0;
   std::vector<CopyRun> copies;
 };
 
@@ -108,6 +110,8 @@
   SliceDev* d_slices = nullptr;
   OpResult* d_results = nullptr;
   OpResult* h_results = nullptr;
+  uint8_t* d_grid = nullptr;
+  int grid = 0;
   bool staged = false;
   uint8_t* d_stage = nullptr;
   std::vector<int> perm;
@@ -148,6 +152,7 @@
   RecvOpDev* h_rop = nullptr;
   SliceDev* h_slices = nullptr;
   OpResult* h_res = nullptr;
+  void* d_grid1 = nullptr;
   uint8_t* bounce_tx = nullptr;
   uint8_t* bounce_rx = nullptr;
   uint64_t bounce_tx_cap = 0, bounce_rx_cap = 0;
@@ -419,6 +424,8 @@
   r.id_pair.clear();
   r.by_qpn.clear();
   cudaFree(r.d_pairs);
+  if (r.d_grid1) cudaFree(r.d_grid1);
+  r.d_grid1 = nullptr;
   cudaFreeHost(r.h_mirrors);
   cudaFreeHost(r.h_sop);
   cudaFreeHost(r.h_rop);
@@ -1328,6 +1335,21 @@
 }
 
 
+static void* grid_work_alloc(size_t bytes) {
+  void* w = nullptr;
+  if (!CU_OK(cudaMalloc(&w, bytes))) return nullptr;
+  if (!CU_OK(cudaMemsetAsync(w, 0, bytes, R().stream)) || !CU_OK(cudaStreamSynchronize(R().stream))) {
+    cudaFree(w);
+    return nullptr;
+  }
+  return w;
+}
+
+static void* single_call_grid_work(Runtime& r) {
+  if (!r.d_grid1) r.d_grid1 = grid_work_alloc(grid_work_bytes(grid_limit()));
+  return r.d_grid1;
+}
+
 static bool ensure_bounce(uint8_t** buf, uint64_t* cap, uint64_t need) {
   if (*cap >= need) return true;
   if (*buf) rt_free(*buf, 1);
@@ -1400,7 +1422,12 @@
   r.h_sop->byte_idx = byte_idx;
   r.h_res->bytes = 0;
   r.h_res->calls = 0;
-  launch_send(r.d_pairs, r.h_sop, r.h_res, 1, r.stream);
+  void* work = single_call_grid_work(r);
+  if (!work) return 0;
+  uint64_t call_bytes = 0;
+  for (size_t i = 0; i < look; i++) call_bytes += slices[i].len;
+  if (call_bytes > p->cap / 2) call_bytes = p->cap / 2;
+  launch_send(r.d_pairs, r.h_sop, r.h_res, 1, grid_for(1, call_bytes), work, r.stream);
   r.launches++;
   if (!CU_OK(cudaGetLastError()) || !CU_OK(cudaStreamSynchronize(r.stream))) {
     p->error = t_err;
@@ -1436,7 +1463,9 @@
   r.h_rop->cap = kcap;
   r.h_res->bytes = 0;
   r.h_res->calls = 0;
-  launch_recv(r.d_pairs, r.h_rop, r.h_res, 1, r.stream);
+  void* work = single_call_grid_work(r);
+  if (!work) return 0;
+  launch_recv(r.d_pairs, r.h_rop, r.h_res, 1, grid_for(1, kcap < p->cap ? kcap : p->cap), work, r.stream);
   r.launches++;
   if (!CU_OK(cudaGetLastError()) || !CU_OK(cudaStreamSynchronize(r.stream))) {
     p->error = t_err;
@@ -1619,6 +1648,33 @@
     }
     ok = ok && CU_OK(cudaMemcpy(b->d_ops, h.data(), sizeof(RecvOpDev) * (nops ? nops : 1), cudaMemcpyHostToDevice));
   }
+  if (ok && nops) {
+    auto op_bytes = [&](int k) -> uint64_t {
+      if (kind == 1) return rops[b->perm[k]].cap;
+      const b200_send_op& o = sops[b->perm[k]];
+      uint64_t t = 0;
+      for (size_t j = 0; j < o.nslices; j++) t += o.slices[j].len;
+      return t;
+    };
+    size_t area = 0;
+    if (b->staged) {
+      for (LanePlan& lp : b->lanes) {
+        if (!lp.nops) continue;
+        uint64_t bytes = 0;
+        for (int k = lp.first_op; k < lp.first_op + lp.nops; k++) bytes += op_bytes(k);
+        lp.grid = grid_for(lp.nops, bytes);
+        lp.grid_off = area;
+        area += grid_work_bytes(lp.grid);
+      }
+    } else {
+      uint64_t bytes = 0;
+      for (int k = 0; k < (int)nops; k++) bytes += op_bytes(k);
+      b->grid = grid_for((int)nops, bytes);
+      area = grid_work_bytes(b->grid);
+    }
+    b->d_grid = (uint8_t*)grid_work_alloc(area);
+    ok = b->d_grid != nullptr;
+  }
   ok = ok && CU_OK(cudaMalloc(&b->d_results, sizeof(OpResult) * (nops ? nops : 1))) &&
        CU_OK(cudaHostAlloc(&b->h_results, sizeof(OpResult) * (nops ? nops : 1), cudaHostAllocPortable));
   if (!ok) {
@@ -1677,8 +1733,8 @@
   }
   if (!b->staged) {
     cudaStream_t s = stream ? (cudaStream_t)stream : r.stream;
-    if (b->kind == 0) launch_send(r.d_pairs, (const SendOpDev*)b->d_ops, b->d_results, b->nops, s);
-    else launch_recv(r.d_pairs, (const RecvOpDev*)b->d_ops, b->d_results, b->nops, s);
+    if (b->kind == 0) launch_send(r.d_pairs, (const SendOpDev*)b->d_ops, b->d_results, b->nops, b->grid, b->d_grid, s);
+    else launch_recv(r.d_pairs, (const RecvOpDev*)b->d_ops, b->d_results, b->nops, b->grid, b->d_grid, s);
     r.launches++;
     return CU_OK(cudaGetLastError()) ? 0 : -1;
   }
@@ -1691,12 +1747,14 @@
       for (const CopyRun& c : lp.copies)
         if (!CU_OK(cudaMemcpyAsync(c.dst, c.src, c.bytes, cudaMemcpyHostToDevice, s))) return -1;
       if (!CU_OK(cudaStreamWaitEvent(s, r.recv_done[L], 0))) return -1;
-      launch_send(r.d_pairs, (const SendOpDev*)b->d_ops + lp.first_op, b->d_results + lp.first_op, lp.nops, s);
+      launch_send(r.d_pairs, (const SendOpDev*)b->d_ops + lp.first_op, b->d_results + lp.first_op, lp.nops, lp.grid,
+                  b->d_grid + lp.grid_off, s);
       if (!CU_OK(cudaEventRecord(r.send_done[L], s))) return -1;
     } else {
       cudaStream_t s = r.lane_down[L];
       if (!CU_OK(cudaStreamWaitEvent(s, r.send_done[L], 0))) return -1;
-      launch_recv(r.d_pairs, (const RecvOpDev*)b->d_ops + lp.first_op, b->d_results + lp.first_op, lp.nops, s);
+      launch_recv(r.d_pairs, (const RecvOpDev*)b->d_ops + lp.first_op, b->d_results + lp.first_op, lp.nops, lp.grid,
+                  b->d_grid + lp.grid_off, s);
       if (!CU_OK(cudaEventRecord(r.recv_done[L], s))) return -1;
       for (const CopyRun& c : lp.copies)
         if (!CU_OK(cudaMemcpyAsync(c.dst, c.src, c.bytes, cudaMemcpyDeviceToHost, s))) return -1;
@@ -1739,6 +1797,7 @@
   rt_free(b->d_slices, 0);
   rt_free(b->d_results, 0);
   rt_free(b->d_stage, 0);
+  rt_free(b->d_grid, 0);
   rt_free(b->h_results, 1);
   delete b;
 }
```

Result: slower. 517.2, median of 6 (-52.4%).
